# TUI-NICR/EMSANet

Hardware: AMD Instinct MI355X
Metric: images/sec (640x480 RGB-D, bs=32/GPU) fwd+bwd (higher is better)
Workload: dtype f32; 1 GPU; BASELINE.json configs[1]: full EMSANet RGB-D (resnet34-NBt1D x2, SE-add fusion, PPM, semantic+instance+orientation+scene heads), 640x480, bs=32/GPU, f32, train mode (BN batch stats, Dropout2d), step = fwd + bwd (fixed output cotangents) + grad all-reduce + SGD-nesterov update at lr 0 (fixed weights) replayed from a hipGraph; global_batch=32, parallelism=dp1, weights=random init (deterministic), mode=train-hipgraph

## Files before the change

emsanet_amd/_lib.py:

```python
import ctypes
import os
from ctypes import POINTER, Structure, c_char_p, c_float, c_int, c_int8, c_int32, c_int64, c_uint32, c_void_p

LIB_PATH = os.environ.get('EMSA_LIB') or os.path.join(
    os.path.dirname(os.path.abspath(__file__)), 'lib', 'libemsanet_hip.so')


class EmsaPackJob(Structure):
    _fields_ = [('src', c_void_p), ('dst0', c_void_p), ('dst1', c_void_p), ('cout', c_int32),
                ('cin', c_int32), ('kh', c_int32), ('kw', c_int32), ('kind', c_int32),
                ('first_block', c_int32), ('cout_total', c_int32), ('cout_off', c_int32),
                ('cin_total', c_int32), ('cin_off', c_int32)]


class EmsaDropoutJob(Structure):
    _fields_ = [('offset', c_int64), ('c', c_int32), ('layer_id', c_uint32), ('p', c_float),
                ('pad_', c_int32)]


class EmsaConvGeom(Structure):
    _fields_ = [
        ('n_img', c_int32),
        ('in_h', c_int32), ('in_w', c_int32),
        ('out_h', c_int32), ('out_w', c_int32),
# ... 63 lines not shown
    'emsa_bn_bwd_reduce_aff_t': (c_int, [c_int32, _P, _P, _P, _P, _P, _P, c_int32, c_int64, c_int32, _P, _P]),
    'emsa_bn_bwd_apply_aff_t': (c_int, [c_int32, _P, _P, _P, _P, _P, _P, _P, _P, c_int32, c_int32, c_int64,
                                        c_int32, _P, _P, _P, _P]),
    'emsa_conv_wgrad_multi_ws_bytes': (c_int64, [c_int32, c_int32, _GP]),
    'emsa_conv_wgrad_multi_t': (c_int, [c_int32, c_int32, _GP, POINTER(c_void_p), POINTER(c_void_p),
                                        POINTER(c_void_p), POINTER(c_void_p), _P, _P]),
    'emsa_pack_wino': (c_int, [_P, _P, _P, c_int32, c_int32, c_int32, _P]),
    'emsa_pack_batch': (c_int, [_P, c_int32, c_int32, _P]),
    'emsa_conv_wino2d_supported': (c_int, [_GP]),
    'emsa_conv_wino2d_stats_rows': (c_int, [_GP]),
    'emsa_conv_wino2d': (c_int, [_GP, _P, _P, _P, _P, _P, _P, _P, _P, c_int32, _P, c_int32, c_int32, _P]),
    'emsa_pack_wino2d': (c_int, [_P, _P, _P, c_int32, c_int32, _P]),
    'emsa_pack_wino2d_packed': (c_int, [_P, _P, c_int32, c_int32, c_int32, _P]),
    'emsa_pack_wino_packed': (c_int, [_P, _P, c_int32, c_int32, c_int32, c_int32, _P]),
    'emsa_conv_wgrad_ws_bytes': (c_int64, [_GP]),
    'emsa_conv_wgrad': (c_int, [_GP, _P, _P, _P, _P, _P, _P]),
    'emsa_pack_weight_fwd': (c_int, [_P, _P] + [c_int32] * 8 + [_P]),
    'emsa_pack_weight_dgrad': (c_int, [_P, _P] + [c_int32] * 8 + [_P]),
    'emsa_unpack_wgrad': (c_int, [_P, _P] + [c_int32] * 8 + [_P]),
    'emsa_pack_weight_pair': (c_int, [_P, _P, _P] + [c_int32] * 4 + [_P]),
    'emsa_stem_pack_input': (c_int, [_P, _P, c_int32, c_int32, c_int32, c_int32, _P]),
    'emsa_stem_pack_weight': (c_int, [_P, _P, c_int32, c_int32, _P]),
    'emsa_stem_pack_input_rows_t': (c_int, [c_int32, _P, _P, c_int32, c_int32, c_int32, _P]),
    'emsa_stem_pack_weight_rows_t': (c_int, [c_int32, _P, _P, c_int32, _P]),
    'emsa_stem_unpack_wgrad_rows': (c_int, [_P, _P, c_int32, _P]),
    'emsa_stem_unpack_wgrad': (c_int, [_P, _P, c_int32, c_int32, _P]),
    'emsa_bn_finalize': (c_int, [_P, c_int32, c_int32, c_int64, _P, _P, c_float, c_float,
                                 _P, _P, _P, _P, _P, _P, _P, _P]),
    'emsa_bn_finalize_ws_bytes': (c_int, [c_int32]),
    'emsa_bn_fold': (c_int, [_P, _P, _P, _P, c_float, c_int32, _P, _P, _P, _P]),
    'emsa_relu_mask_words': (c_int64, [c_int64]),
    'emsa_bn_act_fwd': (c_int, [_P, _P, _P, _P, _P, _P, c_int32, c_int64, c_int32, c_int32, _P,
                                _P]),
    'emsa_bn_bwd_reduce': (c_int, [_P, _P, _P, _P, _P, _P, _P, c_int32, c_int64, c_int32, c_int32,
                                   _P, _P]),
    'emsa_bn_bwd_rows': (c_int, [c_int64, c_int32]),
    'emsa_bn_bwd_apply': (c_int, [_P, _P, _P, _P, _P, _P, _P, _P, _P, c_int32, c_int32, c_int64,
                                  c_int32, c_int32, c_int32, _P, _P, _P, _P, _P]),
    'emsa_dropout2d_mask': (c_int, [_P, c_int32, c_int32, c_float, c_uint32, c_uint32, _P]),
    'emsa_maxpool3x3s2_fwd': (c_int, [_P, _P, _P, c_int32, c_int32, c_int32, c_int32, _P]),
    'emsa_maxpool3x3s2_bwd': (c_int, [_P, _P, _P, c_int32, c_int32, c_int32, c_int32, _P]),
    'emsa_channel_ws_floats': (c_int, [c_int32, c_int64, c_int32]),
    'emsa_channel_mean': (c_int, [_P, _P, _P, c_int32, c_int64, c_int32, _P]),
    'emsa_se_mlp_fwd': (c_int, [_P] * 7 + [c_int32] * 3 + [_P]),
    'emsa_se_mlp_bwd': (c_int, [_P] * 11 + [c_int32] * 3 + [_P]),
    'emsa_se_scale_add_fwd': (c_int, [_P] * 5 + [c_int32, c_int64, c_int32, _P]),
    'emsa_se_scale_bwd_reduce': (c_int, [_P, _P, _P, _P, c_int32, c_int64, c_int32, _P]),
    'emsa_se_scale_bwd_apply': (c_int, [_P] * 5 + [c_int32, c_int64, c_int32, _P]),
    'emsa_up2x_dw3x3_fwd': (c_int, [_P] * 5 + [c_int32] * 4 + [_P]),
    'emsa_up2x_dw3x3_bwd_data': (c_int, [_P] * 3 + [c_int32] * 4 + [_P]),
    'emsa_up2x_dw3x3_bwd_weight': (c_int, [_P] * 4 + [c_int32] * 4 + [_P]),
    'emsa_up2x_dw3x3_bwd': (c_int, [_P] * 6 + [c_int32] * 4 + [_P]),
    'emsa_up2x_dw3x3_bwd_supported': (c_int, [c_int32, c_int32]),
    'emsa_adaptive_avgpool_fwd': (c_int, [_P, _P] + [c_int32] * 5 + [_P]),
    'emsa_adaptive_avgpool_bwd': (c_int, [_P, _P] + [c_int32] * 6 + [_P]),
    'emsa_bilinear_fwd': (c_int, [_P, _P] + [c_int32] * 7 + [_P]),
    'emsa_bilinear_bwd': (c_int, [_P, _P] + [c_int32] * 7 + [_P]),
    'emsa_head_act_fwd': (c_int, [_P, _P, c_int64] + [c_int32] * 5 + [_P]),
    'emsa_head_act_bwd': (c_int, [_P, _P, _P, _P, c_int64] + [c_int32] * 5 + [_P]),
    'emsa_copy_channels': (c_int, [_P, c_int32, _P, c_int32, c_int64, c_int32, _P]),
    'emsa_axpy': (c_int, [_P, _P, c_int64, c_float, _P]),
    'emsa_ce_semantic_blocks': (c_int, [c_int64]),
    'emsa_ce_semantic_fwd': (c_int, [_P, c_int32, _P, _P, c_int32, c_int64, c_float, c_float, _P, _P,
                                     _P]),
    'emsa_ce_semantic_bwd': (c_int, [_P, c_int32, _P, _P, c_int32, c_int64, c_float, c_float, _P, _P,
                                     _P, c_int32, _P]),
    'emsa_softmax_argmax': (c_int, [_P, c_int32, c_int32, c_int64, _P, _P, _P]),
    'emsa_center_candidates_max': (c_int, []),
    'emsa_center_ws_entries': (c_int64, [c_int32, c_int32, c_int32]),
    'emsa_instance_centers': (c_int, [_P, c_int32, c_int32, c_int32, c_int32, c_int32, c_float,
                                      c_int32, _P, _P, _P, _P, _P, _P, _P, _P]),
    'emsa_instance_assign': (c_int, [_P, c_int32, c_int32, c_int32, c_int32, c_float, c_float, _P,
                                     _P, c_int32, _P, c_float, _P, _P]),
    'emsa_panoptic_merge': (c_int, [_P, _P, _P, c_int32, c_int64, c_int32, c_int32, c_int32, _P, _P,
                                    _P, _P, _P, _P]),
    'emsa_instance_stats': (c_int, [_P, _P, _P, c_int32, c_int64, c_int32, _P, _P, _P]),
    'emsa_panoptic_scores': (c_int, [_P, _P, _P, _P, c_int32, c_int64, c_int32, _P, _P, _P, _P, _P, _P,
                                     _P, _P]),
    'emsa_instance_orientation': (c_int, [_P, c_int32, _P, _P, c_int32, c_int64, c_int32, _P, _P, _P]),
    'emsa_confusion_matrix': (c_int, [_P, c_int32, _P, c_int32, c_int64, c_int32, _P, _P, _P]),
    'emsa_panoptic_targets': (c_int, [_P, c_int32, _P, c_int32, _P, c_int32, c_int64, c_int64, _P, _P]),
    'emsa_panoptic_workspace_bytes': (c_int64, [c_int32, c_int32]),
    'emsa_panoptic_pairs': (c_int, [_P, _P, c_int32, c_int64, c_int32, _P, _P, _P]),
    'emsa_panoptic_match': (c_int, [_P, c_int32, c_int32, c_int32, c_int32, c_int64, _P, _P, _P, _P,
                                    _P, _P]),
    'emsa_panoptic_match_pairs': (c_int, [_P, c_int32, c_int32, c_int32, c_int32, c_int64, _P, _P, _P,
                                          _P, _P, _P, _P, _P]),
    'emsa_angular_error': (c_int, [_P, _P, _P, c_int32, c_int32, _P, c_int32, _P, _P, c_int32, c_int64,
                                   _P, _P, _P]),
    'emsa_export_pack': (c_int, [POINTER(EmsaExportJob), c_int32, c_int32, c_int32, c_int32, _P, _P]),
    'emsa_export_instance_ranks': (c_int, [_P, _P, _P, c_int32, c_int32, c_int32, _P, _P, _P, _P, _P,
                                           _P, _P]),
    'emsa_export_instance_masks': (c_int, [_P, c_int32, c_int32, c_int32, c_int32, c_int32, c_int32,
                                           _P, c_int32, _P, _P, c_int32, _P, _P]),
    'emsa_targets_workspace_bytes': (c_int64, [c_int32, c_int32, c_int32]),
    'emsa_targets_table_entries': (c_int, [c_int32]),
    'emsa_targets_stats': (c_int, [_P, c_int32, _P, c_int32, _P, c_int32, c_int32, c_int32, c_int32, _TP,
                                   c_int32, c_int32, _P, _P]),
    'emsa_targets_finalize': (c_int, [c_int32, c_int32, c_int32, _TP, c_int32, c_int32, _P, _P]),
    'emsa_targets_render': (c_int, [_P, c_int32, _P, c_int32, _P, _P, _P, c_int32, c_int32, c_int32,
                                    c_int32, _TP, c_int32, c_int32, c_int32, _P, _P, _P, _P]),
    'emsa_augment_params': (c_int, [_P, _P] + [c_int32] * 7 + [c_int64, c_float, c_float, c_float, _P]),
    'emsa_augment_apply': (c_int, [_P, _P, _P, c_int32, _P, c_int32, _P] + [c_int32] * 5 +
                           [_P, _P, _P, _P, c_float, _P, _P, c_float, c_float, c_int32, c_int32, _P]),
    'emsa_augment_orientations': (c_int, [_P, _P, _P, c_int32, c_int32, _P]),
    'emsa_normal_l1_blocks': (c_int, [c_int64]),
    'emsa_normal_l1_fwd': (c_int, [_P, c_int32, _P, c_int32, c_int64, c_int64, _P, _P, _P]),
    'emsa_normal_l1_bwd': (c_int, [_P, c_int32, _P, c_int32, c_int64, c_int64, _P, _P, _P, c_int32, _P]),
    'emsa_normal_targets': (c_int, [_P, c_int32, c_int32, c_int32, c_int32, POINTER(EmsaNormalScale),
                                    c_int32, _P]),
    'emsa_augment_normal': (c_int, [_P, c_int32, _P] + [c_int32] * 5 + [_P, _P]),
    'emsa_normal_unit': (c_int, [_P, c_int32, c_int64, _P, _P]),
    'emsa_normal_angular_error': (c_int, [_P, c_int32, c_int32, c_int32, c_int32, _P, c_int32, c_int32,
                                          c_int32, _P, _P, _P]),
    'emsa_normalize_rgb': (c_int, [_P, _P, c_int32, c_int32, c_int32, c_float, _P, _P, _P]),
    'emsa_normalize_depth': (c_int, [_P, _P, c_int64, c_float, c_float, c_int32, _P]),
    'emsa_sgd_nesterov': (c_int, [_P, _P, _P, c_int64, c_float, c_float, c_float, c_float, c_int32,
                                  _P]),
    'emsa_add_t': (c_int, [c_int32, _P, _P, _P, c_int64, _P]),
    'emsa_adam_advance': (c_int, [_P, _P, _P]),
    'emsa_adam_step': (c_int, [_P, _P, _P, _P, c_int64, _P, _P, _P]),
    'emsa_instance_loss_blocks': (c_int, [c_int64]),
    'emsa_instance_loss_fwd': (c_int, [_P, c_int32, _P, c_int32, _P, c_int32, _P, _P, _P, _P, _P, _P,
                                       c_int64, c_float, _P, _P, _P]),
    'emsa_instance_loss_bwd': (c_int, [_P, c_int32, _P, c_int32, _P, c_int32, _P, _P, _P, _P, _P, _P,
                                       c_int64, c_float, _P, _P, _P, c_int32, _P, c_int32, _P,
                                       c_int32, _P]),
    'emsa_bn_act_fwd_t': (c_int, [c_int32, _P, _P, _P, _P, _P, _P, c_int32, c_int64, c_int32, c_int32, _P, _P]),
    'emsa_bn_bwd_reduce_t': (c_int, [c_int32, _P, _P, _P, _P, _P, _P, _P, c_int32, c_int64, c_int32, c_int32, _P, _P]),
    'emsa_bn_bwd_apply_t': (c_int, [c_int32, _P, _P, _P, _P, _P, _P, _P, _P, _P, c_int32, c_int32, c_int64, c_int32, c_int32, c_int32, _P, _P, _P, _P, _P]),
    'emsa_maxpool3x3s2_fwd_t': (c_int, [c_int32, _P, _P, _P, c_int32, c_int32, c_int32, c_int32, _P]),
    'emsa_maxpool3x3s2_bwd_t': (c_int, [c_int32, _P, _P, _P, c_int32, c_int32, c_int32, c_int32, _P]),
    'emsa_se_scale_add_fwd_t': (c_int, [c_int32, _P, _P, _P, _P, _P, c_int32, c_int64, c_int32, _P]),
    'emsa_se_scale_bwd_apply_t': (c_int, [c_int32, _P, _P, _P, _P, _P, c_int32, c_int64, c_int32, _P]),
    'emsa_up2x_dw3x3_fwd_t': (c_int, [c_int32, c_int32, _P, _P, _P, _P, _P, c_int32, c_int32, c_int32, c_int32, _P]),
    'emsa_up2x_dw3x3_bwd_data_t': (c_int, [c_int32, c_int32, _P, _P, _P, c_int32, c_int32, c_int32, c_int32, _P]),
    'emsa_up2x_dw3x3_bwd_weight_t': (c_int, [c_int32, c_int32, _P, _P, _P, _P, c_int32, c_int32, c_int32, c_int32, _P]),
    'emsa_up2x_dw3x3_bwd_t': (c_int, [c_int32, c_int32, _P, _P, _P, _P, _P, _P, c_int32, c_int32, c_int32, c_int32, _P]),
    'emsa_adaptive_avgpool_fwd_t': (c_int, [c_int32, _P, _P, c_int32, c_int32, c_int32, c_int32, c_int32, _P]),
    'emsa_adaptive_avgpool_bwd_t': (c_int, [c_int32, _P, _P, c_int32, c_int32, c_int32, c_int32, c_int32, c_int32, _P]),
    'emsa_bilinear_fwd_t': (c_int, [c_int32, _P, _P, c_int32, c_int32, c_int32, c_int32, c_int32, c_int32, c_int32, _P]),
    'emsa_bilinear_bwd_t': (c_int, [c_int32, _P, _P, c_int32, c_int32, c_int32, c_int32, c_int32, c_int32, c_int32, _P]),
    'emsa_nearest_fwd_t': (c_int, [c_int32, _P, _P, c_int32, c_int32, c_int32, c_int32, c_int32, c_int32, c_int32, _P]),
    'emsa_nearest_bwd_t': (c_int, [c_int32, _P, _P, c_int32, c_int32, c_int32, c_int32, c_int32, c_int32, c_int32, _P]),
    'emsa_head_act_fwd_t': (c_int, [c_int32, c_int32, _P, _P, c_int64, c_int32, c_int32, c_int32, c_int32, c_int32, _P]),
    'emsa_head_act_bwd_gather_t': (c_int, [c_int32, _P, c_int32, c_int32, _P, c_int32, c_int32, _P, c_int32,
                                           c_int32, _P, _P, _P, c_int64, c_int32, c_int32, c_int32, c_int32,
                                           c_int32, _P]),
    'emsa_head_act_bwd_t': (c_int, [c_int32, c_int32, _P, _P, _P, _P, c_int64, c_int32, c_int32, c_int32, c_int32, c_int32, _P]),
    'emsa_stem_pack_input_t': (c_int, [c_int32, _P, _P, c_int32, c_int32, c_int32, c_int32, _P]),
    'emsa_channel_mean_t': (c_int, [c_int32, _P, _P, _P, c_int32, c_int64, c_int32, _P]),
    'emsa_se_pair_fwd_t': (c_int, [c_int32] + [_P] * 14 + [c_int32, c_int64, c_int32, c_int32, _P]),
    'emsa_se_scale_bwd_reduce_t': (c_int, [c_int32, _P, _P, _P, _P, c_int32, c_int64, c_int32, _P]),
    'emsa_cast_channels': (c_int, [c_int32, _P, c_int32, c_int32, _P, c_int32, c_int64, c_int32, _P]),
    'emsa_conv_stats_rows_t': (c_int, [c_int32, _GP]),
    'emsa_conv_igemm_t': (c_int, [c_int32, _GP, _P, _P, _P, _P, _P, _P, _P, _P, c_int32, _P, c_int32,
                                  c_int32, _P]),
    'emsa_conv_wgrad_ws_bytes_t': (c_int64, [c_int32, _GP]),
    'emsa_conv_wgrad_t': (c_int, [c_int32, _GP, _P, _P, _P, _P, _P, _P]),
    'emsa_pack_weight_t': (c_int, [c_int32, _P, _P, _P] + [c_int32] * 8 + [_P]),
    'emsa_conv_igemm_splitk_ws_bytes_t': (c_int64, [c_int32, _GP]),
    'emsa_conv_igemm_splitk_t': (c_int, [c_int32, _GP, _P, _P, _P, _P, _P, _P, _P, c_int32, c_int32, _P, _P]),
    'emsa_up2x_dw3x3_fwd_pair_t': (c_int, [c_int32] + [_P] * 10 + [c_int32] * 4 + [_P]),
    'emsa_conv_igemm_pair_t': (c_int, [c_int32, _GP] + [_P] * 14 + [c_int32, c_int32, _P, _P, _P]),
    'emsa_conv_rs_set_cu_budget': (c_int, [c_int32]),
    'emsa_nbt_half_block_supported': (c_int, [c_int32, c_int32, c_int32]),
    'emsa_nbt_half_block_t': (c_int, [c_int32, c_int32, c_int32, c_int32, c_int32, c_int32,
                                      POINTER(c_void_p), c_int32, POINTER(c_void_p), POINTER(c_void_p),
                                      POINTER(c_void_p), POINTER(c_void_p), POINTER(c_void_p),
                                      POINTER(c_void_p), POINTER(c_void_p), c_int32, POINTER(c_void_p),
                                      c_int32, c_int32, _P]),
    'emsa_conv1d_rs_supported': (c_int, [c_int32, _GP]),
    'emsa_conv1d_rs_stats_rows': (c_int, [c_int32, _GP]),
    'emsa_conv1d_rs_t': (c_int, [c_int32, _GP, _P, _P, _P, _P, _P, _P, _P, _P, c_int32, _P, c_int32,
                                 c_int32, _P]),
    'emsa_conv1d_rs_pair_t': (c_int, [c_int32, _GP] + [_P] * 14 + [c_int32, c_int32, _P]),
    'emsa_conv1d_rs_bnb_t': (c_int, [c_int32, _GP, _P, _P, _P, _P, c_int32, _P, c_int32, _P, _P, _P,
                                     _P, _P, c_int32, _P]),
    'emsa_pack_weight_frag_t': (c_int, [c_int32, _P, _P, _P, c_int32, c_int32, _P]),
    'emsa_stem_pack_weight_t': (c_int, [c_int32, _P, _P, c_int32, c_int32, _P]),
    'emsa_dropout2d_mask_dev': (c_int, [_P, c_int32, c_int32, c_float, _P, c_uint32, _P]),
    'emsa_u32_add': (c_int, [_P, c_uint32, _P]),
    'emsa_sgd_nesterov_dev': (c_int, [_P, _P, _P, c_int64, _P, _P]),
    'emsa_prof_enable': (c_int, [c_int32]),
    'emsa_prof_next_flops': (c_int, [ctypes.c_double]),
    'emsa_prof_reset': (c_int, []),
    'emsa_prof_seen': (c_int, [c_int32]),
    'emsa_prof_name': (c_char_p, [c_int32]),
    'emsa_prof_read': (c_int, [c_int32, POINTER(ctypes.c_double), POINTER(ctypes.c_double),
                               POINTER(c_int32)]),
    'emsa_prof_read_bytes': (c_int, [c_int32, POINTER(ctypes.c_double)]),
}

E_SHAPE = -1
_ERR = {-1: 'EMSA_E_SHAPE (unsupported geometry)', -2: 'EMSA_E_ARG (bad argument)',
        -3: 'EMSA_E_LAUNCH (HIP launch failed)'}


class EmsaError(RuntimeError):
    pass


def _load():
    if not os.path.exists(LIB_PATH):
        raise EmsaError(
            f"{LIB_PATH} not found: build the HIP extension first "
            "(python -c 'import __graft_entry__ as g; g.build()' or make -C emsanet_amd/csrc). "
            "There is no CPU / torch fallback for the EMSANet engine.")
    import torch
    lib = ctypes.CDLL(LIB_PATH)
    for name, (res, args) in SIGNATURES.items():
        fn = getattr(lib, name)
        fn.restype = res
        fn.argtypes = args
    return lib


_lib = None


def lib():
    global _lib
    if _lib is None:
        _lib = _load()
    return _lib


def check(status, name):
    if status != 0:
        raise EmsaError(f"{name} failed: {_ERR.get(status, status)}")
```

emsanet_amd/csrc/pointwise.hip:

```cpp
#include <type_traits>

#include <cstdlib>

#include <atomic>
#include "common.h"

namespace {

constexpr int kThreads = 256;
#ifndef EMSA_PW_BLOCKS_PER_CU
#define EMSA_PW_BLOCKS_PER_CU 8
#endif
constexpr int kMaxBlocks = 256 * EMSA_PW_BLOCKS_PER_CU;

inline int grid_for(long work_items) {
  long b = (work_items + kThreads - 1) / kThreads;
  if (b < 1) b = 1;
  if (b > kMaxBlocks) b = kMaxBlocks;
  return (int)b;
}

__global__ void pack_weight_kernel(const float* __restrict__ src, float* __restrict__ dst, int cout,
                                   int cin, int kh, int kw, int cout_total, int cout_off,
                                   int cin_total, int cin_off, int mode,
                                   float* __restrict__ dst2 = nullptr) {
  const long total = (long)cout * cin * kh * kw;
  const int taps = kh * kw;
  for (long i = blockIdx.x * (long)blockDim.x + threadIdx.x; i < total;
       i += (long)gridDim.x * blockDim.x) {
    const int tap = (int)(i % taps);
    const long r = i / taps;
    const int ci = (int)(r % cin), co = (int)(r / cin);
    if (mode == 3) {
      const float v = src[i];
      dst[((long)tap * cout_total + cout_off + co) * cin_total + cin_off + ci] = v;
      dst2[((long)tap * cin_total + cin_off + ci) * cout_total + cout_off + co] = v;
    } else if (mode == 0) {
      dst[((long)tap * cout_total + cout_off + co) * cin_total + cin_off + ci] = src[i];
    } else if (mode == 1) {
      dst[((long)tap * cin_total + cin_off + ci) * cout_total + cout_off + co] = src[i];
    } else {
      dst[i] = src[((long)tap * cout_total + cout_off + co) * cin_total + cin_off + ci];
    }
  }
}

template <typename T>
__global__ void pack_weight_t_kernel(const float* __restrict__ src, T* __restrict__ dst,
                                     T* __restrict__ dst2, int cout, int cin, int taps,
                                     int cout_total, int cout_off, int cin_total, int cin_off) {
  const long total = (long)cout * cin * taps;
  for (long i = blockIdx.x * (long)blockDim.x + threadIdx.x; i < total;
       i += (long)gridDim.x * blockDim.x) {
    const int tap = (int)(i % taps);
    const long r = i / taps;
    const int ci = (int)(r % cin), co = (int)(r / cin);
    const float v = src[i];
    if (dst) emsa_st1(dst + ((long)tap * cout_total + cout_off + co) * cin_total + cin_off + ci, v);
    if (dst2) emsa_st1(dst2 + ((long)tap * cin_total + cin_off + ci) * cout_total + cout_off + co, v);
  }
}

template <typename T>
__global__ void stem_pack_input_kernel(const float* __restrict__ x, T* __restrict__ y, int n,
                                       int c, int h, int w) {
  const int wp = w + 8;
  const long total = (long)n * h * wp;
  for (long i = blockIdx.x * (long)blockDim.x + threadIdx.x; i < total;
       i += (long)gridDim.x * blockDim.x) {
    const int col = (int)(i % wp);
    const long r = i / wp;
    const int row = (int)(r % h), img = (int)(r / h);
    const int sw = col - 3;
    float4 v = emsa_zero4();
    if (sw >= 0 && sw < w) {
      const long base = ((long)img * c * h + row) * w + sw;
      const long plane = (long)h * w;
      v.x = x[base];
      if (c > 1) v.y = x[base + plane];
      if (c > 2) v.z = x[base + 2 * plane];
      if (c > 3) v.w = x[base + 3 * plane];
    }
    emsa_st4(y + i * 4, v);
  }
}

template <typename T>
__global__ void stem_pack_input_rows_kernel(const float* __restrict__ x, T* __restrict__ y, int n,
                                            int h, int w) {
  const int wp = w + 8, hp = h + 4;
  const long total = (long)n * hp * wp;
  for (long i = blockIdx.x * (long)blockDim.x + threadIdx.x; i < total;
       i += (long)gridDim.x * blockDim.x) {
    const int col = (int)(i % wp);
    const long r = i / wp;
    const int row = (int)(r % hp), img = (int)(r / hp);
    const int sw = col - 3;
    float v[4] = {0.f, 0.f, 0.f, 0.f};
    if (sw >= 0 && sw < w) {
#pragma unroll
      for (int k = 0; k < 4; ++k) {
        const int sr = row - 3 + k;
        if (sr >= 0 && sr < h) v[k] = x[((long)img * h + sr) * w + sw];
      }
    }
    emsa_st4(y + i * 4, make_float4(v[0], v[1], v[2], v[3]));
  }
}
template <typename T>
__global__ void stem_pack_weight_rows_kernel(const float* __restrict__ w, T* __restrict__ wp,
                                             int cout, int unpack) {
  const int total = 2 * cout * 32;
  for (int i = blockIdx.x * blockDim.x + threadIdx.x; i < total; i += gridDim.x * blockDim.x) {
    const int k = i % 32, co = (i / 32) % cout, t = i / (32 * cout);
    const int kw = k / 4, kh = 4 * t + (k % 4);
    const bool real = kw < 7 && kh < 7;
    if (!unpack) {
      emsa_st1(wp + i, real ? w[(co * 7 + kh) * 7 + kw] : 0.f);
    } else if (real) {
      emsa_st1(wp + (co * 7 + kh) * 7 + kw, w[i]);
    }
  }
}

template <typename T>
__global__ void stem_pack_weight_kernel(const float* __restrict__ w, T* __restrict__ wp,
                                        int cout, int cin, int unpack) {
  const int total = 7 * cout * 32;
  for (int i = blockIdx.x * blockDim.x + threadIdx.x; i < total; i += gridDim.x * blockDim.x) {
    const int k = i % 32, co = (i / 32) % cout, kh = i / (32 * cout);
    const int kw = k / 4, c = k % 4;
    const bool real = kw < 7 && c < cin;
    if (!unpack) {
      emsa_st1(wp + i, real ? w[((co * cin + c) * 7 + kh) * 7 + kw] : 0.f);
    } else if (real) {
      emsa_st1(wp + ((co * cin + c) * 7 + kh) * 7 + kw, w[i]);
    }
  }
}

constexpr int kBnSlices = 64;
__global__ void bn_partial_kernel(const float* __restrict__ stats, int rows, int c,
                                  double* __restrict__ ws) {
  __shared__ double sh[3][8][32];
  const int cl = threadIdx.x & 31, rg = threadIdx.x >> 5;
  const int ch = blockIdx.x * 32 + cl;
  const int slices = gridDim.y, sl = blockIdx.y;
  const int per = (rows + slices - 1) / slices;
  const int r0 = sl * per, r1 = min(r0 + per, rows);
  double s0 = 0.0, s1 = 0.0, q = 0.0;
  if (ch < c)
    for (int r = r0 + rg; r < r1; r += 8) {
      const double nb = (double)stats[((long)2 * rows + r) * c + ch];
      if (nb > 0.0) {
        const double sb = (double)stats[((long)0 * rows + r) * c + ch];
        s0 += nb;
        s1 += sb;
        q += (double)stats[((long)1 * rows + r) * c + ch] + sb * sb / nb;
      }
    }
  sh[0][rg][cl] = s0; sh[1][rg][cl] = s1; sh[2][rg][cl] = q;
  __syncthreads();
  if (rg == 0 && ch < c) {
    s0 = s1 = q = 0.0;
#pragma unroll
    for (int k = 0; k < 8; ++k) { s0 += sh[0][k][cl]; s1 += sh[1][k][cl]; q += sh[2][k][cl]; }
    double* o = ws + ((long)sl * c + ch) * 3;
    o[0] = s0; o[1] = s1; o[2] = q;
  }
}

__global__ void bn_finalize_kernel(const double* __restrict__ ws, int slices, int c,
                                   const float* __restrict__ gamma, const float* __restrict__ beta,
                                   float eps, float momentum, float* running_mean,
                                   float* running_var, float* __restrict__ scale,
                                   float* __restrict__ shift, float* __restrict__ save_mean,
                                   float* __restrict__ save_invstd) {
  __shared__ double sh[3][8][32];
  const int cl = threadIdx.x & 31, rg = threadIdx.x >> 5;
  const int ch = blockIdx.x * 32 + cl;
  double n = 0.0, s1 = 0.0, q = 0.0;
  if (ch < c)
    for (int sl = rg; sl < slices; sl += 8) {
      const double* o = ws + ((long)sl * c + ch) * 3;
      n += o[0]; s1 += o[1]; q += o[2];
    }
  sh[0][rg][cl] = n; sh[1][rg][cl] = s1; sh[2][rg][cl] = q;
  __syncthreads();
  if (rg != 0 || ch >= c) return;
  n = s1 = q = 0.0;
#pragma unroll
  for (int k = 0; k < 8; ++k) { n += sh[0][k][cl]; s1 += sh[1][k][cl]; q += sh[2][k][cl]; }
  const double mean = n > 0.0 ? s1 / n : 0.0;
  double m2 = q - s1 * mean;
  if (m2 < 0.0) m2 = 0.0;
  const double var = n > 0.0 ? m2 / n : 0.0;
  const float invstd = (float)(1.0 / sqrt(var + (double)eps));
  const float sc = gamma[ch] * invstd;
  scale[ch] = sc;
  shift[ch] = beta[ch] - (float)mean * sc;
  save_mean[ch] = (float)mean;
  save_invstd[ch] = invstd;
  if (running_mean) {
    const double unbiased = n > 1.0 ? m2 / (n - 1.0) : var;
    running_mean[ch] = (1.f - momentum) * running_mean[ch] + momentum * (float)mean;
    running_var[ch] = (1.f - momentum) * running_var[ch] + momentum * (float)unbiased;
  }
}

template <int RG>
__global__ __launch_bounds__(4 * RG) void bn_finalize_rows_kernel(const float* __restrict__ stats, int rows, int c,
                                        const float* __restrict__ gamma, const float* __restrict__ beta,
                                        float eps, float momentum, float* running_mean,
                                        float* running_var, float* __restrict__ scale,
                                        float* __restrict__ shift, float* __restrict__ save_mean,
                                        float* __restrict__ save_invstd) {
  __shared__ double sh[3][RG][4];
  const int cl = threadIdx.x & 3, rg = threadIdx.x >> 2;
  const int ch = blockIdx.x * 4 + cl;
  const int chc = ch < c ? ch : c - 1;
  double n = 0.0, s1 = 0.0, q = 0.0;
#pragma unroll 8
  for (int r = rg; r < rows; r += RG) {
    const float nbf = stats[((long)2 * rows + r) * c + chc];
    const float sbf = stats[((long)0 * rows + r) * c + chc];
    const float m2f = stats[((long)1 * rows + r) * c + chc];
    const double nb = (double)nbf, sb = (double)sbf;
    const bool ok = nbf > 0.f;
    n += ok ? nb : 0.0;
    s1 += ok ? sb : 0.0;
    const double r0 = (double)(1.0f / (ok ? nbf : 1.f));
    const double rn = r0 * (2.0 - (ok ? nb : 1.0) * r0);
    q += ok ? (double)m2f + sb * sb * rn : 0.0;
  }
#pragma unroll
  for (int off = 4; off < 64; off <<= 1) {
    n += __shfl_xor(n, off);
    s1 += __shfl_xor(s1, off);
    q += __shfl_xor(q, off);
  }
  constexpr int NW = 4 * RG / 64;
  const int wv = threadIdx.x >> 6;
  if ((threadIdx.x & 63) < 4) { sh[0][wv][cl] = n; sh[1][wv][cl] = s1; sh[2][wv][cl] = q; }
  __syncthreads();
  if (rg != 0 || ch >= c) return;
  n = s1 = q = 0.0;
#pragma unroll
  for (int k = 0; k < NW; ++k) { n += sh[0][k][cl]; s1 += sh[1][k][cl]; q += sh[2][k][cl]; }
  const double mean = n > 0.0 ? s1 / n : 0.0;
  double m2 = q - s1 * mean;
  if (m2 < 0.0) m2 = 0.0;
  const double var = n > 0.0 ? m2 / n : 0.0;
  const float invstd = (float)(1.0 / sqrt(var + (double)eps));
  const float sc = gamma[ch] * invstd;
  scale[ch] = sc;
  shift[ch] = beta[ch] - (float)mean * sc;
  save_mean[ch] = (float)mean;
  save_invstd[ch] = invstd;
  if (running_mean) {
    const double unbiased = n > 1.0 ? m2 / (n - 1.0) : var;
    running_mean[ch] = (1.f - momentum) * running_mean[ch] + momentum * (float)mean;
    running_var[ch] = (1.f - momentum) * running_var[ch] + momentum * (float)unbiased;
  }
}

__global__ void bn_fold_kernel(const float* gamma, const float* beta, const float* rm,
                               const float* rv, float eps, int c, float* scale, float* shift,
                               float* invstd) {
  const int i = blockIdx.x * blockDim.x + threadIdx.x;
  if (i < c) {
    const float is = 1.0f / sqrtf(rv[i] + eps);
    const float sc = gamma[i] * is;
    scale[i] = sc;
    shift[i] = beta[i] - rm[i] * sc;
    if (invstd) invstd[i] = is;
  }
}

__device__ __forceinline__ float bn_mul(float a, float b) {
#pragma clang fp contract(off)
  return a * b;
}
__device__ __forceinline__ float bn_add(float a, float b) {
#pragma clang fp contract(off)
  return a + b;
}
__device__ __forceinline__ float bn_affine(float x, float sc, float sh) { return __builtin_fmaf(x, sc, sh); }
__device__ __forceinline__ float bn_acc_xhat(float acc, float g, float x, float mu, float is) {
  return __builtin_fmaf(bn_mul(g, bn_add(x, -mu)), is, acc);
}
__device__ __forceinline__ float bn_dx_train(float g, float x, float mu, float is, float gi, float db,
                                             float dg, float inv_count) {
  const float xh = bn_mul(bn_add(x, -mu), is);
  const float t = __builtin_fmaf(-db, inv_count, g);
  return bn_mul(gi, __builtin_fmaf(-bn_mul(xh, dg), inv_count, t));
}

template <typename T> struct VecIO {
  static constexpr int V = 8;
  typedef typename std::conditional<std::is_same<T, emsa_f16>::value, _Float16, __bf16>::type E;
  typedef E ev __attribute__((ext_vector_type(8)));
  typedef float fv __attribute__((ext_vector_type(8)));
  static __device__ __forceinline__ void load(const T* p, float (&v)[8]) {
    const fv f = __builtin_convertvector(*reinterpret_cast<const ev*>(p), fv);
#pragma unroll
    for (int k = 0; k < 8; ++k) v[k] = f[k];
  }
  typedef ev raw;
  static __device__ __forceinline__ raw load_raw(const T* p) { return *reinterpret_cast<const ev*>(p); }
  static __device__ __forceinline__ void cvt(const raw& r, float (&v)[8]) {
    const fv f = __builtin_convertvector(r, fv);
#pragma unroll
    for (int k = 0; k < 8; ++k) v[k] = f[k];
  }
  static __device__ __forceinline__ void store(T* p, const float (&v)[8]) {
    fv f;
#pragma unroll
    for (int k = 0; k < 8; ++k) f[k] = v[k];
    *reinterpret_cast<ev*>(p) = __builtin_convertvector(f, ev);
  }
};
template <> struct VecIO<float> {
  static constexpr int V = 4;
  static __device__ __forceinline__ void load(const float* p, float (&v)[4]) {
    const float4 f = emsa_ld4(p);
    v[0] = f.x; v[1] = f.y; v[2] = f.z; v[3] = f.w;
  }
  typedef float4 raw;
  static __device__ __forceinline__ raw load_raw(const float* p) { return emsa_ld4(p); }
  static __device__ __forceinline__ void cvt(const raw& f, float (&v)[4]) {
    v[0] = f.x; v[1] = f.y; v[2] = f.z; v[3] = f.w;
  }
  static __device__ __forceinline__ void store(float* p, const float (&v)[4]) {
    emsa_st4(p, make_float4(v[0], v[1], v[2], v[3]));
  }
};
template <int V>
__device__ __forceinline__ void ldf(const float* p, float (&v)[V]) {
#pragma unroll
  for (int k = 0; k < V; k += 4) {
    const float4 f = emsa_ld4(p + k);
    v[k] = f.x; v[k + 1] = f.y; v[k + 2] = f.z; v[k + 3] = f.w;
  }
}

template <typename T>
__global__ void bn_act_fwd_kernel(const T* __restrict__ x, T* __restrict__ y,
                                  const float* __restrict__ scale, const float* __restrict__ shift,
                                  const float* __restrict__ drop,
                                  const T* __restrict__ residual, long hw, int cvn, long totalv,
                                  int act, uint64_t* __restrict__ mask_bits) {
  constexpr int V = VecIO<T>::V;
  for (long i = blockIdx.x * (long)blockDim.x + threadIdx.x; i < totalv;
       i += (long)gridDim.x * blockDim.x) {
    const int cv = (int)(i % cvn);
    const long pix = i / cvn;
    float v[V], sc[V], sh[V];
    VecIO<T>::load(x + i * V, v);
    ldf<V>(scale + cv * V, sc);
    ldf<V>(shift + cv * V, sh);
#pragma unroll
    for (int k = 0; k < V; ++k) v[k] = bn_affine(v[k], sc[k], sh[k]);
    if (drop) {
      float d[V];
      ldf<V>(drop + (pix / hw) * (long)cvn * V + cv * V, d);
#pragma unroll
      for (int k = 0; k < V; ++k) v[k] = bn_mul(v[k], d[k]);
    }
    if (residual) {
      float r[V];
      VecIO<T>::load(residual + i * V, r);
#pragma unroll
      for (int k = 0; k < V; ++k) v[k] = bn_add(v[k], r[k]);
    }
    if (act == EMSA_ACT_RELU) {
#pragma unroll
      for (int k = 0; k < V; ++k) v[k] = fmaxf(v[k], 0.f);
    }
    VecIO<T>::store(y + i * V, v);
    if (mask_bits) {
      uint64_t b[V];
#pragma unroll
      for (int k = 0; k < V; ++k) b[k] = __ballot(v[k] > 0.f);
      if ((i & 63) == 0) {
        uint64_t* m = mask_bits + (i >> 6) * V;
#pragma unroll
        for (int k = 0; k < V; ++k) m[k] = b[k];
      }
    }
  }
}

template <typename T, bool DROP, bool RES>
__global__ __launch_bounds__(kThreads) void bn_act_fwd_fast_kernel(
    const T* __restrict__ x, T* __restrict__ y, const float* __restrict__ scale,
    const float* __restrict__ shift, const float* __restrict__ drop, const T* __restrict__ residual,
    uint32_t hw, int cvn_log2, uint32_t totalv, int act, uint64_t* __restrict__ mask_bits) {
  constexpr int V = VecIO<T>::V;
  typedef typename VecIO<T>::raw Raw;
  const uint32_t stride = gridDim.x * kThreads;
  uint32_t i = blockIdx.x * kThreads + threadIdx.x;
  const uint32_t cvn = 1u << cvn_log2, cv = i & (cvn - 1);
  const uint32_t dpix = stride >> cvn_log2;
  uint32_t pix = i >> cvn_log2;
  float sc[V], sh[V];
  ldf<V>(scale + cv * V, sc);
  ldf<V>(shift + cv * V, sh);
  auto finish = [&](uint32_t idx, const Raw& rx, const Raw& rr, const float (&d)[V]) {
    float v[V];
    VecIO<T>::cvt(rx, v);
#pragma unroll
    for (int k = 0; k < V; ++k) v[k] = bn_affine(v[k], sc[k], sh[k]);
    if constexpr (DROP) {
#pragma unroll
      for (int k = 0; k < V; ++k) v[k] = bn_mul(v[k], d[k]);
    }
    if constexpr (RES) {
      float r[V];
      VecIO<T>::cvt(rr, r);
#pragma unroll
      for (int k = 0; k < V; ++k) v[k] = bn_add(v[k], r[k]);
    }
    if (act == EMSA_ACT_RELU) {
#pragma unroll
      for (int k = 0; k < V; ++k) v[k] = fmaxf(v[k], 0.f);
    }
    VecIO<T>::store(y + (size_t)idx * V, v);
    if (mask_bits) {
      uint64_t b[V];
#pragma unroll
      for (int k = 0; k < V; ++k) b[k] = __ballot(v[k] > 0.f);
      if ((idx & 63) == 0) {
        uint64_t* m = mask_bits + (size_t)(idx >> 6) * V;
#pragma unroll
        for (int k = 0; k < V; ++k) m[k] = b[k];
      }
    }
  };
  auto ld_drop = [&](uint32_t px, float (&d)[V]) {
    if constexpr (DROP) ldf<V>(drop + ((size_t)(px / hw) * cvn + cv) * V, d);
  };
  uint32_t iw = i & ~63u;
  for (; iw + stride + 64 <= totalv; iw += 2 * stride, i += 2 * stride, pix += 2 * dpix) {
    const uint32_t i1 = i + stride;
    const Raw x0 = VecIO<T>::load_raw(x + (size_t)i * V);
    const Raw x1 = VecIO<T>::load_raw(x + (size_t)i1 * V);
    Raw r0 = x0, r1 = x1;
    if constexpr (RES) {
// ... 2325 lines not shown
    case EMSA_DT_F32: { return maxpool3x3s2_fwd_impl<float>((const float*)x, (float*)y, idx, n, h, w, c, stream); }
    case EMSA_DT_BF16: { return maxpool3x3s2_fwd_impl<emsa_bf16>((const emsa_bf16*)x, (emsa_bf16*)y, idx, n, h, w, c, stream); }
    case EMSA_DT_F16: { return maxpool3x3s2_fwd_impl<emsa_f16>((const emsa_f16*)x, (emsa_f16*)y, idx, n, h, w, c, stream); }
    default: return EMSA_E_ARG;
  }
}
template <typename T>
static int maxpool3x3s2_bwd_impl(const T* dy, const int8_t* idx, T* dx, int32_t n, int32_t h, int32_t w, int32_t c, void* stream) {
  if (!dy || !dx || !idx) return EMSA_E_ARG;
  if (!cv_ok<T>(c)) return EMSA_E_SHAPE;
  constexpr int V = VecIO<T>::V;
  const long total = (long)n * ((h + 1) / 2) * ((w + 1) / 2) * (c / V);
  if (idx32_ok((long)n * h * w * c))
    hipLaunchKernelGGL((maxpool_bwd_kernel<T, uint32_t>), dim3(grid_for(total)), dim3(kThreads), 0,
                       (hipStream_t)stream, dy, idx, dx, n, h, w, c / V);
  else
    hipLaunchKernelGGL((maxpool_bwd_kernel<T, long>), dim3(grid_for(total)), dim3(kThreads), 0,
                       (hipStream_t)stream, dy, idx, dx, n, h, w, c / V);
  return emsa_launch_status();
}
extern "C" int emsa_maxpool3x3s2_bwd(const float* dy, const int8_t* idx, float* dx, int32_t n, int32_t h, int32_t w, int32_t c, void* stream) {
  return maxpool3x3s2_bwd_impl<float>(dy, idx, dx, n, h, w, c, stream);
}
extern "C" int emsa_maxpool3x3s2_bwd_t(int32_t dtype, const void* dy, const int8_t* idx, void* dx, int32_t n, int32_t h, int32_t w, int32_t c, void* stream) {
  switch (dtype) {
    case EMSA_DT_F32: { return maxpool3x3s2_bwd_impl<float>((const float*)dy, idx, (float*)dx, n, h, w, c, stream); }
    case EMSA_DT_BF16: { return maxpool3x3s2_bwd_impl<emsa_bf16>((const emsa_bf16*)dy, idx, (emsa_bf16*)dx, n, h, w, c, stream); }
    case EMSA_DT_F16: { return maxpool3x3s2_bwd_impl<emsa_f16>((const emsa_f16*)dy, idx, (emsa_f16*)dx, n, h, w, c, stream); }
    default: return EMSA_E_ARG;
  }
}

static std::atomic<int> g_batch_invariant{0};
static int channel_splits(long hw, int n) {
  int splits = (int)((hw + 511) / 512);
  if (splits > 64) splits = 64;
  if ((long)n * splits <= 64 && !g_batch_invariant.load(std::memory_order_relaxed)) {
    splits = (int)((hw + 63) / 64);
    if (splits > 256) splits = 256;
  }
  if (splits < 1) splits = 1;
  return splits;
}

extern "C" int emsa_set_batch_invariant(int on) {
  return g_batch_invariant.exchange(on ? 1 : 0, std::memory_order_relaxed);
}

template <typename T>
static int channel_dot(const T* a, const T* b, float* out, float* ws, int n, long hw,
                       int c, float scale, hipStream_t st) {
  if (!cv_ok<T>(c)) return EMSA_E_SHAPE;
  const int splits = channel_splits(hw, n);
  const int cvn = c / VecIO<T>::V;
  if (cvn > kThreads) {
    const dim3 grid(n * splits, (cvn + kThreads - 1) / kThreads);
    if (b)
      hipLaunchKernelGGL((channel_dot_wide_kernel<T, true>), grid, dim3(kThreads), 0, st, a, b, ws, hw,
                         cvn, splits);
    else
      hipLaunchKernelGGL((channel_dot_wide_kernel<T, false>), grid, dim3(kThreads), 0, st, a, b, ws, hw,
                         cvn, splits);
    hipLaunchKernelGGL(channel_dot_finish_kernel, dim3((n * c + 255) / 256), dim3(256), 0, st, ws,
                       out, n, c, splits, scale);
    return emsa_launch_status();
  }
  const int lanes = kThreads / cvn;
  const size_t lds = (size_t)lanes * c * sizeof(float);
  if (b)
    hipLaunchKernelGGL((channel_dot_kernel<T, true>), dim3(n * splits), dim3(kThreads), lds, st, a, b,
                       ws, hw, cvn, splits);
  else
    hipLaunchKernelGGL((channel_dot_kernel<T, false>), dim3(n * splits), dim3(kThreads), lds, st, a, b,
                       ws, hw, cvn, splits);
  hipLaunchKernelGGL(channel_dot_finish_kernel, dim3((n * c + 255) / 256), dim3(256), 0, st, ws,
                     out, n, c, splits, scale);
  return emsa_launch_status();
}

extern "C" int emsa_channel_ws_floats(int32_t n, int64_t hw, int32_t c) {
  return n * channel_splits((long)hw, n) * c;
}
extern "C" int emsa_channel_mean(const float* x, float* gap, float* ws, int32_t n, int64_t hw,
                                 int32_t c, void* stream) {
  if (!x || !gap || !ws) return EMSA_E_ARG;
  return channel_dot<float>(x, nullptr, gap, ws, n, (long)hw, c, 1.0f / (float)hw,
                            (hipStream_t)stream);
}
extern "C" int emsa_channel_mean_t(int32_t dtype, const void* x, float* gap, float* ws, int32_t n,
                                   int64_t hw, int32_t c, void* stream) {
  if (!x || !gap || !ws) return EMSA_E_ARG;
  EMSA_DISPATCH_DTYPE(dtype, T, return channel_dot<T>((const T*)x, (const T*)nullptr, gap, ws, n,
                                                      (long)hw, c, 1.0f / (float)hw,
                                                      (hipStream_t)stream));
  return EMSA_E_ARG;
}
extern "C" int emsa_se_scale_bwd_reduce(const float* dout, const float* x, float* ds, float* ws,
                                        int32_t n, int64_t hw, int32_t c, void* stream) {
  if (!dout || !x || !ds || !ws) return EMSA_E_ARG;
  return channel_dot<float>(dout, x, ds, ws, n, (long)hw, c, 1.0f, (hipStream_t)stream);
}
extern "C" int emsa_se_scale_bwd_reduce_t(int32_t dtype, const void* dout, const void* x, float* ds,
                                          float* ws, int32_t n, int64_t hw, int32_t c,
                                          void* stream) {
  if (!dout || !x || !ds || !ws) return EMSA_E_ARG;
  EMSA_DISPATCH_DTYPE(dtype, T, return channel_dot<T>((const T*)dout, (const T*)x, ds, ws, n,
                                                      (long)hw, c, 1.0f, (hipStream_t)stream));
  return EMSA_E_ARG;
}

extern "C" int emsa_se_mlp_fwd(const float* gap, const float* w1, const float* b1,
                               const float* w2, const float* b2, float* hid, float* s, int32_t n,
                               int32_t c, int32_t cr, void* stream) {
  if (!gap || !w1 || !b1 || !w2 || !b2 || !hid || !s) return EMSA_E_ARG;
  hipLaunchKernelGGL(se_mlp_fwd_kernel, dim3(n), dim3(256), (size_t)(c + cr) * sizeof(float),
                     (hipStream_t)stream, gap, w1, b1, w2, b2, hid, s, c, cr);
  return emsa_launch_status();
}
template <typename T>
static int se_pair_fwd(const T* xa, const T* xb, float* ws, const float* const* wts, float* gap,
                       float* hid, float* s, int n, long hw, int c, int cr, hipStream_t st) {
  if (!cv_ok<T>(c)) return EMSA_E_SHAPE;
  const int splits = channel_splits(hw, n);
  const int cvn = c / VecIO<T>::V;
  if (cvn > kThreads) {
    hipLaunchKernelGGL((channel_dot_wide_kernel<T, false>),
                       dim3(2 * n * splits, (cvn + kThreads - 1) / kThreads), dim3(kThreads), 0, st, xa,
                       (const T*)nullptr, ws, hw, cvn, splits, xb, n * splits);
  } else {
    const int lanes = kThreads / cvn;
    const size_t lds = (size_t)lanes * c * sizeof(float);
    hipLaunchKernelGGL((channel_dot_kernel<T, false>), dim3(2 * n * splits), dim3(kThreads), lds, st, xa,
                       (const T*)nullptr, ws, hw, cvn, splits, xb, n * splits);
  }
  hipLaunchKernelGGL(se_mlp_pair_fwd_kernel, dim3(2 * n), dim3(256),
                     (size_t)(c + cr) * sizeof(float), st, ws, splits, 1.0f / (float)hw, wts[0],
                     wts[1], wts[2], wts[3], wts[4], wts[5], wts[6], wts[7], gap, hid, s, n, c, cr);
  return emsa_launch_status();
}
extern "C" int emsa_se_pair_fwd_t(int32_t dtype, const void* xa, const void* xb, float* ws,
                                  const float* w1a, const float* b1a, const float* w2a,
                                  const float* b2a, const float* w1b, const float* b1b,
                                  const float* w2b, const float* b2b, float* gap, float* hid,
                                  float* s, int32_t n, int64_t hw, int32_t c, int32_t cr,
                                  void* stream) {
  if (!xa || !xb || !ws || !w1a || !b1a || !w2a || !b2a || !w1b || !b1b || !w2b || !b2b || !gap ||
      !hid || !s)
    return EMSA_E_ARG;
  const float* wts[8] = {w1a, b1a, w2a, b2a, w1b, b1b, w2b, b2b};
  EMSA_DISPATCH_DTYPE(dtype, T, return se_pair_fwd<T>((const T*)xa, (const T*)xb, ws, wts, gap, hid,
                                                      s, n, (long)hw, c, cr, (hipStream_t)stream));
  return EMSA_E_ARG;
}
extern "C" int emsa_se_mlp_bwd(const float* gap, const float* w1, const float* w2,
                               const float* hid, const float* s, const float* ds, float* dgap,
                               float* dw1, float* db1, float* dw2, float* db2, int32_t n,
                               int32_t c, int32_t cr, void* stream) {
  if (!gap || !w1 || !w2 || !hid || !s || !ds || !dgap || !dw1 || !db1 || !dw2 || !db2)
    return EMSA_E_ARG;
  hipStream_t st = (hipStream_t)stream;
  if (n <= c && cr <= 32 && cr >= 1) {
    float* dz1 = dw2;
    const size_t lds = (size_t)(c + (256 / cr) * cr + cr) * sizeof(float);
    hipLaunchKernelGGL(se_mlp_bwd_a_kernel, dim3(n), dim3(256), lds, st, w1, w2, hid, s, ds, dgap,
                       dz1, c, cr);
    const int wblocks = (c * cr + 255) / 256;
    hipLaunchKernelGGL(se_mlp_bwd_w_kernel<0>, dim3(wblocks + (cr + 255) / 256), dim3(256), 0, st,
                       gap, hid, s, ds, dz1, dw1, db1, n, c, cr, wblocks);
    hipLaunchKernelGGL(se_mlp_bwd_w_kernel<1>, dim3(wblocks + (c + 255) / 256), dim3(256), 0, st,
                       gap, hid, s, ds, dz1, dw2, db2, n, c, cr, wblocks);
    return emsa_launch_status();
  }
  if ((size_t)n * cr * sizeof(float) > 60000) return EMSA_E_SHAPE;
  hipLaunchKernelGGL(se_mlp_bwd_kernel, dim3(8), dim3(256), (size_t)n * cr * sizeof(float), st, gap,
                     w1, w2, hid, s, ds, dgap, dw1, db1, dw2, db2, n, c, cr);
  return emsa_launch_status();
}

template <typename T>
static int se_scale_add_fwd_impl(const T* a, const float* sa, const T* b, const float* sb, T* out, int32_t n, int64_t hw, int32_t c, void* stream) {
  if (!a || !sa || !out || ((b == nullptr) != (sb == nullptr))) return EMSA_E_ARG;
  if (!cv_ok<T>(c)) return EMSA_E_SHAPE;
  const long totalv = (long)n * hw * (c / VecIO<T>::V);
  const dim3 grid(grid_for(totalv)), block(kThreads);
  hipStream_t st = (hipStream_t)stream;
  const int cvn = c / VecIO<T>::V;
#define EMSA_SE_FWD(B, I)                                                                          \
  hipLaunchKernelGGL((se_scale_add_fwd_kernel<T, B, I>), grid, block, 0, st, a, sa, b, sb, out,   \
                     (I)hw, cvn, (I)totalv)
  if (idx32_ok((long)n * hw * c)) {
    if (b) EMSA_SE_FWD(true, uint32_t); else EMSA_SE_FWD(false, uint32_t);
  } else {
    if (b) EMSA_SE_FWD(true, long); else EMSA_SE_FWD(false, long);
  }
#undef EMSA_SE_FWD
  return emsa_launch_status();
}
extern "C" int emsa_se_scale_add_fwd(const float* a, const float* sa, const float* b, const float* sb, float* out, int32_t n, int64_t hw, int32_t c, void* stream) {
  return se_scale_add_fwd_impl<float>(a, sa, b, sb, out, n, hw, c, stream);
}
extern "C" int emsa_se_scale_add_fwd_t(int32_t dtype, const void* a, const float* sa, const void* b, const float* sb, void* out, int32_t n, int64_t hw, int32_t c, void* stream) {
  switch (dtype) {
    case EMSA_DT_F32: { return se_scale_add_fwd_impl<float>((const float*)a, sa, (const float*)b, sb, (float*)out, n, hw, c, stream); }
    case EMSA_DT_BF16: { return se_scale_add_fwd_impl<emsa_bf16>((const emsa_bf16*)a, sa, (const emsa_bf16*)b, sb, (emsa_bf16*)out, n, hw, c, stream); }
    case EMSA_DT_F16: { return se_scale_add_fwd_impl<emsa_f16>((const emsa_f16*)a, sa, (const emsa_f16*)b, sb, (emsa_f16*)out, n, hw, c, stream); }
    default: return EMSA_E_ARG;
  }
}
template <typename T>
static int se_scale_bwd_apply_impl(const T* dout, const float* s, const float* dgap, const T* dx_extra, T* dx, int32_t n, int64_t hw, int32_t c, void* stream) {
  if (!dout || !s || !dgap || !dx) return EMSA_E_ARG;
  if (!cv_ok<T>(c)) return EMSA_E_SHAPE;
  const long totalv = (long)n * hw * (c / VecIO<T>::V);
  const dim3 grid(grid_for(totalv)), block(kThreads);
  hipStream_t st = (hipStream_t)stream;
  const int cvn = c / VecIO<T>::V;
  const float inv_hw = 1.0f / (float)hw;
#define EMSA_SE_BWD(E, I)                                                                          \
  hipLaunchKernelGGL((se_scale_bwd_apply_kernel<T, E, I>), grid, block, 0, st, dout, s, dgap,     \
                     dx_extra, dx, (I)hw, cvn, (I)totalv, inv_hw)
  if (idx32_ok((long)n * hw * c)) {
    if (dx_extra) EMSA_SE_BWD(true, uint32_t); else EMSA_SE_BWD(false, uint32_t);
  } else {
    if (dx_extra) EMSA_SE_BWD(true, long); else EMSA_SE_BWD(false, long);
  }
#undef EMSA_SE_BWD
  return emsa_launch_status();
}
extern "C" int emsa_se_scale_bwd_apply(const float* dout, const float* s, const float* dgap, const float* dx_extra, float* dx, int32_t n, int64_t hw, int32_t c, void* stream) {
  return se_scale_bwd_apply_impl<float>(dout, s, dgap, dx_extra, dx, n, hw, c, stream);
}
extern "C" int emsa_se_scale_bwd_apply_t(int32_t dtype, const void* dout, const float* s, const float* dgap, const void* dx_extra, void* dx, int32_t n, int64_t hw, int32_t c, void* stream) {
  switch (dtype) {
    case EMSA_DT_F32: { return se_scale_bwd_apply_impl<float>((const float*)dout, s, dgap, (const float*)dx_extra, (float*)dx, n, hw, c, stream); }
    case EMSA_DT_BF16: { return se_scale_bwd_apply_impl<emsa_bf16>((const emsa_bf16*)dout, s, dgap, (const emsa_bf16*)dx_extra, (emsa_bf16*)dx, n, hw, c, stream); }
    case EMSA_DT_F16: { return se_scale_bwd_apply_impl<emsa_f16>((const emsa_f16*)dout, s, dgap, (const emsa_f16*)dx_extra, (emsa_f16*)dx, n, hw, c, stream); }
    default: return EMSA_E_ARG;
  }
}

template <typename T, typename TO>
static int up2x_dw3x3_fwd_impl(const T* x, const float* wdw, const float* bias, const T* skip, TO* y, int32_t n, int32_t h, int32_t w, int32_t c, void* stream) {
  if (!x || !wdw || !y) return EMSA_E_ARG;
  if (!c4_ok(c)) return EMSA_E_SHAPE;
  const long total = (long)n * 4 * h * w * (c / 4);
  static const int nt_env = [] {
    const char* e = getenv("EMSA_UP2X_NT");
    return e ? (e[0] == '1' ? 1 : 0) : -1;
  }();
  const bool nt = nt_env >= 0 ? nt_env == 1 : c >= 32;
  const dim3 grid(grid_for(total)), block(kThreads);
  const size_t lds = (size_t)9 * c * sizeof(float);
  hipStream_t st = (hipStream_t)stream;
#define EMSA_UP_FWD(NTF, I)                                                                         \
  do {                                                                                              \
    if (skip)                                                                                       \
      hipLaunchKernelGGL((up2x_dw_fwd_kernel<T, TO, NTF, I, true>), grid, block, lds, st, x, wdw,   \
                         bias, skip, y, n, h, w, c / 4);                                            \
    else                                                                                            \
      hipLaunchKernelGGL((up2x_dw_fwd_kernel<T, TO, NTF, I, false>), grid, block, lds, st, x, wdw,  \
                         bias, skip, y, n, h, w, c / 4);                                            \
  } while (0)
  const bool i32 = idx32_ok((long)n * 4 * h * w * c);
  if (nt && std::is_same<TO, float>::value) {
    if (i32) EMSA_UP_FWD(true, uint32_t); else EMSA_UP_FWD(true, long);
  } else {
    if (i32) EMSA_UP_FWD(false, uint32_t); else EMSA_UP_FWD(false, long);
  }
#undef EMSA_UP_FWD
  return emsa_launch_status();
}
template <typename T>
static int up2x_pair_impl(const T* x0, const T* x1, const float* w0, const float* w1, const float* b0,
                          const float* b1, const T* s0, const T* s1, T* y0, T* y1, int n, int h,
                          int w, int c, hipStream_t st) {
  const long total = (long)n * 4 * h * w * (c / 4);
  if ((s0 == nullptr) != (s1 == nullptr)) return EMSA_E_ARG;
#define EMSA_UP_PAIR(I, SK)                                                                         \
  hipLaunchKernelGGL((up2x_dw_fwd_kernel<T, T, false, I, SK>), dim3(grid_for(total), 2),            \
                     dim3(kThreads), (size_t)9 * c * sizeof(float), st, x0, w0, b0, s0, y0, n, h, w, \
                     c / 4, x1, w1, b1, s1, y1)
  if (idx32_ok((long)n * 4 * h * w * c)) {
    if (s0) EMSA_UP_PAIR(uint32_t, true); else EMSA_UP_PAIR(uint32_t, false);
  } else {
    if (s0) EMSA_UP_PAIR(long, true); else EMSA_UP_PAIR(long, false);
  }
#undef EMSA_UP_PAIR
  return emsa_launch_status();
}
extern "C" int emsa_up2x_dw3x3_fwd_pair_t(int32_t dtype, const void* x0, const void* x1,
                                          const float* wdw0, const float* wdw1, const float* bias0,
                                          const float* bias1, const void* skip0, const void* skip1,
                                          void* y0, void* y1, int32_t n, int32_t h, int32_t w,
                                          int32_t c, void* stream) {
  if (!x0 || !x1 || !wdw0 || !wdw1 || !y0 || !y1 || y0 == y1) return EMSA_E_ARG;
  if ((bias0 == nullptr) != (bias1 == nullptr) || (skip0 == nullptr) != (skip1 == nullptr))
    return EMSA_E_ARG;
  if (!c4_ok(c)) return EMSA_E_SHAPE;
  hipStream_t st = (hipStream_t)stream;
  if (dtype == EMSA_DT_BF16)
    return up2x_pair_impl<emsa_bf16>((const emsa_bf16*)x0, (const emsa_bf16*)x1, wdw0, wdw1, bias0, bias1,
                                     (const emsa_bf16*)skip0, (const emsa_bf16*)skip1, (emsa_bf16*)y0,
                                     (emsa_bf16*)y1, n, h, w, c, st);
  if (dtype == EMSA_DT_F16)
    return up2x_pair_impl<emsa_f16>((const emsa_f16*)x0, (const emsa_f16*)x1, wdw0, wdw1, bias0, bias1,
                                    (const emsa_f16*)skip0, (const emsa_f16*)skip1, (emsa_f16*)y0,
// ... 457 lines not shown
```

emsanet_amd/functional.py:

```python
import ctypes
import os

import torch

from . import _lib
from ._lib import EmsaConvGeom, check

ACT_NONE, ACT_RELU = 0, 1


def _stream():
    return torch.cuda.current_stream().cuda_stream


_POISON = bool(os.environ.get('EMSA_POISON'))


def _empty(shape, device, dtype=torch.float32):
    t = torch.empty(shape, device=device, dtype=dtype)
    if _POISON:
        t.fill_(float('nan') if dtype.is_floating_point else 111)
    return t


# ... 990 lines not shown
    y = act_empty(n, c, h, w, x.device, dtype=x.dtype)
    L = _lib.lib()
    bits = None
    if want_mask and act == ACT_RELU:
        bits = torch.empty(L.emsa_relu_mask_words(n * c * h * w), device=x.device,
                           dtype=torch.int64)
    check(call_t('emsa_bn_act_fwd', dt(x), _p(x), _p(y), _p(scale), _p(shift), _p(drop),
                 _p(residual), n, h * w, c, act, _p(bits), _stream()), 'emsa_bn_act_fwd')
    return (y, bits) if want_mask else y


def bn_bwd(dy, y, x, gamma, mean, invstd, drop, act, train, want_dres, dg_out=None, db_out=None):
    n, c, h, w = x.shape
    assert ld_of(x) == c and ld_of(dy) == c and dy.dtype == x.dtype
    L = _lib.lib()
    code = dt(x)
    bits = None
    if y is not None and y.dtype == torch.int64:
        y, bits = None, y
    rows = L.emsa_bn_bwd_rows(n * h * w, c)
    partial = _empty((2, rows, c), x.device)
    check(call_t('emsa_bn_bwd_reduce', code, _p(dy), _p(y), _p(bits), _p(x), _p(mean), _p(invstd),
                 _p(drop), n, h * w, c, act, _p(partial), _stream()), 'emsa_bn_bwd_reduce')
    dx = act_empty(n, c, h, w, x.device, dtype=x.dtype)
    dres = act_empty(n, c, h, w, x.device, dtype=x.dtype) if want_dres else None
    if dg_out is None or db_out is None:
        dgb = _empty((2, c), x.device)
        dg_out, db_out = dgb[0], dgb[1]
    check(call_t('emsa_bn_bwd_apply', code, _p(dy), _p(y), _p(bits), _p(x), _p(gamma), _p(mean),
                 _p(invstd), _p(drop), _p(partial), rows, n, h * w, c, act, 1 if train else 0,
                 _p(dx), _p(dres), _p(dg_out), _p(db_out), _stream()), 'emsa_bn_bwd_apply')
    return dx, dres, dg_out, db_out


def dropout2d_mask(n, c, p, seed, layer_id, device):
    m = _empty((n, c), device)
    if torch.is_tensor(seed):
        check(_lib.lib().emsa_dropout2d_mask_dev(_p(m), n, c, p, _p(seed), layer_id, _stream()),
              'emsa_dropout2d_mask_dev')
    else:
        check(_lib.lib().emsa_dropout2d_mask(_p(m), n, c, p, seed & 0xFFFFFFFF, layer_id,
                                             _stream()), 'emsa_dropout2d_mask')
    return m


def dropout2d_mask_batch(jobs_dev, n_jobs, total_floats, n, max_c, seed, device):
    m = _empty((total_floats,), device)
    if torch.is_tensor(seed):
        check(_lib.lib().emsa_dropout2d_mask_batch(_p(m), _p(jobs_dev), n_jobs, n, max_c, 0, _p(seed),
                                                   _stream()), 'emsa_dropout2d_mask_batch')
    else:
        check(_lib.lib().emsa_dropout2d_mask_batch(_p(m), _p(jobs_dev), n_jobs, n, max_c,
                                                   seed & 0xFFFFFFFF, None, _stream()),
              'emsa_dropout2d_mask_batch')
    return m


def maxpool_fwd(x):
    n, c, h, w = x.shape
    assert ld_of(x) == c
    oh, ow = (h + 1) // 2, (w + 1) // 2
    y = act_empty(n, c, oh, ow, x.device, dtype=x.dtype)
    idx = _empty((n, oh, ow, c), x.device, torch.int8)
    check(call_t('emsa_maxpool3x3s2_fwd', dt(x), _p(x), _p(y), _p(idx), n, h, w, c, _stream()),
          'emsa_maxpool3x3s2_fwd')
    return y, idx


def maxpool_bwd(dy, idx, in_hw):
    n, c = dy.shape[:2]
    h, w = in_hw
    assert ld_of(dy) == c
    dx = act_empty(n, c, h, w, dy.device, dtype=dy.dtype)
    check(call_t('emsa_maxpool3x3s2_bwd', dt(dy), _p(dy), _p(idx), _p(dx), n, h, w, c, _stream()),
          'emsa_maxpool3x3s2_bwd')
    return dx


def channel_mean(x):
    n, c, h, w = x.shape
    assert ld_of(x) == c
    gap = _empty((n, c), x.device)
    ws = _empty((_lib.lib().emsa_channel_ws_floats(n, h * w, c),), x.device)
    check(call_t('emsa_channel_mean', dt(x), _p(x), _p(gap), _p(ws), n, h * w, c, _stream()),
          'emsa_channel_mean')
    return gap


def se_mlp_fwd(gap, w1, b1, w2, b2):
    n, c = gap.shape
    cr = w1.shape[0]
    hid = _empty((n, cr), gap.device)
    s = _empty((n, c), gap.device)
    check(_lib.lib().emsa_se_mlp_fwd(_p(gap), _p(w1), _p(b1), _p(w2), _p(b2), _p(hid), _p(s), n, c,
                                     cr, _stream()), 'emsa_se_mlp_fwd')
    return hid, s


def se_pair_fwd(xa, xb, wa, wb):
    n, c, h, w = xa.shape
    assert xb.shape == xa.shape and xb.dtype == xa.dtype and ld_of(xa) == c and ld_of(xb) == c
    cr = wa[0].shape[0]
    dev = xa.device
    gap, hid, s = _empty((2, n, c), dev), _empty((2, n, cr), dev), _empty((2, n, c), dev)
    ws = _empty((2 * _lib.lib().emsa_channel_ws_floats(n, h * w, c),), dev)
    check(_lib.lib().emsa_se_pair_fwd_t(dt(xa), _p(xa), _p(xb), _p(ws), _p(wa[0]), _p(wa[1]),
                                        _p(wa[2]), _p(wa[3]), _p(wb[0]), _p(wb[1]), _p(wb[2]),
                                        _p(wb[3]), _p(gap), _p(hid), _p(s), n, h * w, c, cr,
                                        _stream()), 'emsa_se_pair_fwd_t')
    return gap[0], gap[1], hid[0], hid[1], s[0], s[1]


def se_mlp_bwd(gap, w1, w2, hid, s, ds):
    n, c = gap.shape
    cr = w1.shape[0]
    dev = gap.device
    dgap = _empty((n, c), dev)
    dw1 = _empty((cr, c), dev)
    db1 = _empty((cr,), dev)
    dw2 = _empty((c, cr), dev)
    db2 = _empty((c,), dev)
    check(_lib.lib().emsa_se_mlp_bwd(_p(gap), _p(w1), _p(w2), _p(hid), _p(s), _p(ds), _p(dgap),
                                     _p(dw1), _p(db1), _p(dw2), _p(db2), n, c, cr, _stream()),
          'emsa_se_mlp_bwd')
    return dgap, dw1, db1, dw2, db2


def se_scale_add(a, sa, b=None, sb=None):
    n, c, h, w = a.shape
    out = act_empty(n, c, h, w, a.device, dtype=a.dtype)
    check(call_t('emsa_se_scale_add_fwd', dt(a), _p(a), _p(sa), _p(b), _p(sb), _p(out), n, h * w,
                 c, _stream()), 'emsa_se_scale_add_fwd')
    return out


def se_scale_bwd_reduce(dout, x):
    n, c, h, w = x.shape
    assert dout.dtype == x.dtype
    ds = _empty((n, c), x.device)
    ws = _empty((_lib.lib().emsa_channel_ws_floats(n, h * w, c),), x.device)
    check(call_t('emsa_se_scale_bwd_reduce', dt(x), _p(dout), _p(x), _p(ds), _p(ws), n, h * w, c,
                 _stream()), 'emsa_se_scale_bwd_reduce')
    return ds


def se_scale_bwd_apply(dout, s, dgap, extra=None):
    n, c, h, w = dout.shape
    dx = act_empty(n, c, h, w, dout.device, dtype=dout.dtype)
    check(call_t('emsa_se_scale_bwd_apply', dt(dout), _p(dout), _p(s), _p(dgap), _p(extra), _p(dx),
                 n, h * w, c, _stream()), 'emsa_se_scale_bwd_apply')
    return dx


def _two(name, feat, out_f32, *args):
    code = dt(feat)
    L = _lib.lib()
    if code == 0:
        return getattr(L, name)(*args)
    return getattr(L, name + '_t')(code, 1 if out_f32 else 0, *args)


def up2x_dw_fwd(x, wdw, bias, skip=None, out_f32=False):
    n, c, h, w = x.shape
    assert ld_of(x) == c and (skip is None or (ld_of(skip) == c and skip.dtype == x.dtype))
    y = act_empty(n, c, 2 * h, 2 * w, x.device,
                  dtype=torch.float32 if out_f32 else x.dtype)
    check(_two('emsa_up2x_dw3x3_fwd', x, out_f32, _p(x), _p(wdw), _p(bias), _p(skip), _p(y), n, h,
               w, c, _stream()), 'emsa_up2x_dw3x3_fwd')
    return y


UP2X_FUSED_BWD = os.environ.get('EMSA_UP2X_FUSED', '1') != '0'


def up2x_dw_fwd_pair(xs, wdws, biases, skips):
    x0, x1 = xs
    if x0.dtype == torch.float32 or x0.dtype != x1.dtype or x0.shape != x1.shape:
        return None
    if (biases[0] is None) != (biases[1] is None) or (skips[0] is None) != (skips[1] is None):
        return None
    n, c, h, w = x0.shape
    for t in (x0, x1) + tuple(k for k in skips if k is not None):
        if ld_of(t) != c or t.dtype != x0.dtype:
            return None
    y0 = act_empty(n, c, 2 * h, 2 * w, x0.device, dtype=x0.dtype)
    y1 = act_empty(n, c, 2 * h, 2 * w, x0.device, dtype=x0.dtype)
    check(_lib.lib().emsa_up2x_dw3x3_fwd_pair_t(
        dt(x0), _p(x0), _p(x1), _p(wdws[0]), _p(wdws[1]), _p(biases[0]), _p(biases[1]), _p(skips[0]),
        _p(skips[1]), _p(y0), _p(y1), n, h, w, c, _stream()), 'emsa_up2x_dw3x3_fwd_pair_t')
    return y0, y1


def up2x_dw_bwd(dy, x, wdw, need_dx=True):
    n, c, h, w = x.shape
    assert ld_of(dy) == c
    out_f32 = dy.dtype == torch.float32
    if not out_f32 and dy.dtype != x.dtype:
        raise _lib.EmsaError(f"up-sampling gradient {dy.dtype} for {x.dtype} features")
    dx = act_empty(n, c, h, w, x.device, dtype=x.dtype) if need_dx else None
    dwb = torch.zeros(c * 10, device=x.device, dtype=torch.float32)
    dw, db = dwb[:c * 9], dwb[c * 9:]
    if UP2X_FUSED_BWD and _lib.lib().emsa_up2x_dw3x3_bwd_supported(c, x.element_size()):
        check(_two('emsa_up2x_dw3x3_bwd', x, out_f32, _p(dy), _p(x), _p(wdw), _p(dx), _p(dw), _p(db),
                   n, h, w, c, _stream()), 'emsa_up2x_dw3x3_bwd')
        return dx, dw, db
    if need_dx:
        check(_two('emsa_up2x_dw3x3_bwd_data', x, out_f32, _p(dy), _p(wdw), _p(dx), n, h, w, c,
                   _stream()), 'emsa_up2x_dw3x3_bwd_data')
    check(_two('emsa_up2x_dw3x3_bwd_weight', x, out_f32, _p(dy), _p(x), _p(dw), _p(db), n, h, w, c,
               _stream()), 'emsa_up2x_dw3x3_bwd_weight')
    return dx, dw, db


def adaptive_avgpool_fwd(x, bins):
    n, c, h, w = x.shape
    assert ld_of(x) == c
    y = act_empty(n, c, bins, bins, x.device, dtype=x.dtype)
    check(call_t('emsa_adaptive_avgpool_fwd', dt(x), _p(x), _p(y), n, h, w, c, bins, _stream()),
          'emsa_adaptive_avgpool_fwd')
    return y


def adaptive_avgpool_bwd(dy, dx, bins, accumulate):
    n, c, h, w = dx.shape
    assert dy.dtype == dx.dtype
    check(call_t('emsa_adaptive_avgpool_bwd', dt(dx), _p(dy), _p(dx), n, h, w, c, bins,
                 1 if accumulate else 0, _stream()), 'emsa_adaptive_avgpool_bwd')
    return dx


def bilinear_fwd(x, out):
    n, c, ih, iw = x.shape
    oh, ow = out.shape[2:]
    assert ld_of(x) == c and out.dtype == x.dtype
    check(call_t('emsa_bilinear_fwd', dt(x), _p(x), _p(out), n, ih, iw, oh, ow, c, ld_of(out),
                 _stream()), 'emsa_bilinear_fwd')
    return out


def bilinear_bwd(dy, in_hw):
    n, c, oh, ow = dy.shape
    ih, iw = in_hw
    dx = act_empty(n, c, ih, iw, dy.device)
    check(call_t('emsa_bilinear_bwd', dt(dy), _p(dy), _p(dx), n, ih, iw, oh, ow, c, ld_of(dy),
                 _stream()), 'emsa_bilinear_bwd')
    if dy.dtype != torch.float32:
        dx = cast(dx, dy.dtype)
    return dx


def nearest_fwd(x, out):
    n, c, ih, iw = x.shape
    oh, ow = out.shape[2:]
    assert ld_of(x) == c and out.dtype == x.dtype
    check(_lib.lib().emsa_nearest_fwd_t(dt(x), _p(x), _p(out), n, ih, iw, oh, ow, c, ld_of(out),
                                        _stream()), 'emsa_nearest_fwd_t')
    return out


def nearest_bwd(dy, in_hw):
    n, c, oh, ow = dy.shape
    ih, iw = in_hw
    dx = act_empty(n, c, ih, iw, dy.device)
    check(_lib.lib().emsa_nearest_bwd_t(dt(dy), _p(dy), _p(dx), n, ih, iw, oh, ow, c, ld_of(dy),
                                        _stream()), 'emsa_nearest_bwd_t')
    if dy.dtype != torch.float32:
        dx = cast(dx, dy.dtype)
    return dx


def add(a, b):
    assert a.shape == b.shape and a.dtype == b.dtype and ld_of(a) == a.shape[1] == ld_of(b)
    n, c, h, w = a.shape
    out = act_empty(n, c, h, w, a.device, dtype=a.dtype)
    check(_lib.lib().emsa_add_t(dt(a), _p(a), _p(b), _p(out), a.numel(), _stream()), 'emsa_add_t')
    return out


def head_act_fwd(x, n_sig, n_tanh, n_norm=0, norm_off=3):
    n, c, h, w = x.shape
    assert ld_of(x) == c
    y = act_empty(n, c, h, w, x.device)
    check(_two('emsa_head_act_fwd', x, True, _p(x), _p(y), n * h * w, c, n_sig, n_tanh, norm_off,
               n_norm, _stream()), 'emsa_head_act_fwd')
    return y


def head_act_bwd(dy, y, n_sig, n_tanh, n_norm=0, x=None, norm_off=3, dtype=torch.float32):
    n, c, h, w = y.shape
    assert ld_of(dy) == c and dy.dtype == torch.float32 and y.dtype == torch.float32
    dx = act_empty(n, c, h, w, y.device, dtype=dtype)
    check(_two('emsa_head_act_bwd', dx, True, _p(dy), _p(y), _p(x), _p(dx), n * h * w, c, n_sig,
               n_tanh, norm_off, n_norm, _stream()), 'emsa_head_act_bwd')
    return dx


HEAD_GATHER = os.environ.get('EMSA_HEAD_GATHER', '1') != '0'


def head_act_bwd_gather(grads, sizes, y, n_sig, n_tanh, n_norm=0, x=None, norm_off=3,
                        dtype=torch.float32):
    n, c, h, w = y.shape
    if c != 8 or len(sizes) > 3 or y.dtype != torch.float32 or ld_of(y) != c or not HEAD_GATHER:
        return None
    gs = []
    for g_ in grads:
# ... 41 lines not shown
```

emsanet_amd/nn.py:

```python
import os

import torch
import torch.nn as nn

from . import functional as Fn
from . import ops
from .functional import ACT_NONE, ACT_RELU


class Spec:
    BLOCK_BN_EPS = 1e-3
    DEFAULT_BN_EPS = 1e-5
    BN_MOMENTUM = 0.1
    SE_REDUCTION = 16
    PPM_BINS = (1, 5)
    STEM_BIAS = False
    DW_UPSAMPLE_BIAS = True
    SIDE_OUTPUT_KERNEL = 1
    SKIP_FUSION_1X1 = True
    ORIENTATION_L2_NORMALIZE = False
    RESNET_LAYERS = {'resnet18': (2, 2, 2, 2), 'resnet34': (3, 4, 6, 3), 'resnet50': (3, 4, 6, 3),
                     'resnet101': (3, 4, 23, 3)}


# ... 2 lines not shown


class ConvNormAct(nn.Module):

    def __init__(self, cin, cout, kernel_size, stride=1, act=True, eps=Spec.DEFAULT_BN_EPS):
        super().__init__()
        self.conv = nn.Conv2d(cin, cout, kernel_size, stride=stride, padding=kernel_size // 2,
                              bias=False)
        self.norm = nn.BatchNorm2d(cout, eps=eps, momentum=Spec.BN_MOMENTUM)
        self.act = ACT_RELU if act else ACT_NONE
        self._crt, self._brt = ops.ConvRT(self.conv), ops.BNRT(self.norm)

    def forward(self, x):
        if _fast_eval(self):
            return ops.conv_bn_act_eval(Fn.as_act(x), self._crt, self._brt, self.act)
        return ops.ConvBNActFunction.apply(x, self._crt, self._brt, self.act, self.conv.weight,
                                           self.norm.weight, self.norm.bias)


class Dropout2dHash(nn.Module):

    def __init__(self, p):
        super().__init__()
        self.p = float(p)
        self.layer_id = -1
        self.seed_fn = lambda: 0

    def mask(self, n, c, device):
        if not self.training or self.p == 0.0:
            return None
        pre = getattr(self, '_premade', None)
        if pre is not None and pre.shape == (n, c) and pre.device == device:
            self._premade = None
            return pre
        return Fn.dropout2d_mask(n, c, self.p, self.seed_fn(), self.layer_id, device)


class NonBottleneck1D(nn.Module):
    def __init__(self, cin, cout, stride=1, dropout_p=0.0):
        super().__init__()
        self.conv3x1_1 = nn.Conv2d(cin, cout, (3, 1), stride=(stride, 1), padding=(1, 0))
        self.conv1x3_1 = nn.Conv2d(cout, cout, (1, 3), stride=(1, stride), padding=(0, 1))
        self.bn1 = nn.BatchNorm2d(cout, eps=Spec.BLOCK_BN_EPS, momentum=Spec.BN_MOMENTUM)
        self.conv3x1_2 = nn.Conv2d(cout, cout, (3, 1), padding=(1, 0))
        self.conv1x3_2 = nn.Conv2d(cout, cout, (1, 3), padding=(0, 1))
        self.bn2 = nn.BatchNorm2d(cout, eps=Spec.BLOCK_BN_EPS, momentum=Spec.BN_MOMENTUM)
        self.dropout = Dropout2dHash(dropout_p)
        if stride != 1 or cin != cout:
            self.downsample = nn.Sequential(
                nn.Conv2d(cin, cout, 1, stride=stride, bias=False),
                nn.BatchNorm2d(cout, eps=Spec.DEFAULT_BN_EPS, momentum=Spec.BN_MOMENTUM))
        else:
            self.downsample = None
        self._rt = ops.NBt1DRT(self)

    def forward(self, x):
        if _fast_eval(self):
            return ops.nbt1d_eval(Fn.as_act(x, dense=True), self._rt)
        drop = self.dropout.mask(x.shape[0], self.conv1x3_2.out_channels, x.device)
        return ops.NBt1DFunction.apply(x, self._rt, drop, *self._rt.params())


class _ResidualBlock(nn.Module):

    def _add(self, name, cin, cout, k, stride=1):
        conv = nn.Conv2d(cin, cout, k, stride=stride, padding=k // 2, bias=False)
        bn = nn.BatchNorm2d(cout, eps=Spec.DEFAULT_BN_EPS, momentum=Spec.BN_MOMENTUM)
        setattr(self, f'conv{name}', conv)
        setattr(self, f'bn{name}', bn)
        rt = (ops.ConvRT(conv), ops.BNRT(bn), conv, bn)
        self._crts.append(rt[0])
        return rt

    def _finish(self, cin, cout, stride):
        if stride != 1 or cin != cout:
            self.downsample = nn.Sequential(
                nn.Conv2d(cin, cout, 1, stride=stride, bias=False),
                nn.BatchNorm2d(cout, eps=Spec.DEFAULT_BN_EPS, momentum=Spec.BN_MOMENTUM))
            self._ds = (ops.ConvRT(self.downsample[0]), ops.BNRT(self.downsample[1]),
                        self.downsample[0], self.downsample[1])
            self._crts.append(self._ds[0])
        else:
            self.downsample, self._ds = None, None

    def forward(self, x):
        fast = _fast_eval(self)
        x = Fn.as_act(x, dense=True) if fast else x
        y = x
        for crt, brt, conv, bn in self._chain[:-1]:
            y = ops.conv_bn_act_eval(y, crt, brt, ACT_RELU) if fast else \
                ops.ConvBNActFunction.apply(y, crt, brt, ACT_RELU, conv.weight, bn.weight, bn.bias)
        idn = x
        if self._ds is not None:
            crt, brt, conv, bn = self._ds
            idn = ops.conv_bn_act_eval(x, crt, brt, ACT_NONE) if fast else \
                ops.ConvBNActFunction.apply(x, crt, brt, ACT_NONE, conv.weight, bn.weight, bn.bias)
        crt, brt, conv, bn = self._chain[-1]
        if fast:
            return ops.conv_bn_act_eval(y, crt, brt, ACT_RELU, residual=idn)
        return ops.ConvBNAddActFunction.apply(y, idn, crt, brt, ACT_RELU, conv.weight, bn.weight,
                                              bn.bias)


class BasicBlock(_ResidualBlock):
    expansion = 1

    def __init__(self, cin, c, stride=1, dropout_p=0.0):
        super().__init__()
        self._crts = []
        self._chain = [self._add('1', cin, c, 3, stride), self._add('2', c, c, 3)]
        self._finish(cin, c, stride)


class Bottleneck(_ResidualBlock):
    expansion = 4

    def __init__(self, cin, c, stride=1, dropout_p=0.0):
        super().__init__()
        self._crts = []
        self._chain = [self._add('1', cin, c, 1), self._add('2', c, c, 3, stride),
                       self._add('3', c, 4 * c, 1)]
        self._finish(cin, 4 * c, stride)


RESNET_BLOCKS = {'nonbottleneck1d': None, 'basicblock': BasicBlock, 'bottleneck': Bottleneck}


class ResNetNBt1D(nn.Module):

    def __init__(self, name, n_input_channels, dropout_p, block='nonbottleneck1d'):
        super().__init__()
        if name not in Spec.RESNET_LAYERS:
            raise NotImplementedError(f"backbone '{name}' (ResNet-18/34/101 layouts)")
        if block not in RESNET_BLOCKS:
            raise NotImplementedError(f"resnet block '{block}'")
        layers = Spec.RESNET_LAYERS[name]
        self.conv1 = nn.Conv2d(n_input_channels, 64, 7, stride=2, padding=3, bias=Spec.STEM_BIAS)
        self.bn1 = nn.BatchNorm2d(64, eps=Spec.DEFAULT_BN_EPS, momentum=Spec.BN_MOMENTUM)
        cin = 64
        cls = RESNET_BLOCKS[block] or NonBottleneck1D
        exp = getattr(cls, 'expansion', 1)
        for i, (c, n) in enumerate(zip((64, 128, 256, 512), layers)):
            blocks = []
            for j in range(n):
                blocks.append(cls(cin, c, stride=2 if (i > 0 and j == 0) else 1,
                                  dropout_p=dropout_p))
                cin = c * exp
            setattr(self, f'layer{i + 1}', nn.Sequential(*blocks))
        self.stage_channels = (64, 64 * exp, 128 * exp, 256 * exp, 512 * exp)
        self.stage_downsamplings = (2, 4, 8, 16, 32)
        self._stem = ops.StemRT(self.conv1, self.bn1)
        self.compute_dtype = torch.float32

    def forward_stage(self, i, x):
        if i == 0:
            if _fast_eval(self):
                return ops.stem_eval(x, self._stem, self.compute_dtype)
            return ops.StemFunction.apply(x, self._stem, self.conv1.weight, self.bn1.weight,
                                          self.bn1.bias, self.conv1.bias, self.compute_dtype)
        if i == 1:
            x = ops.MaxPoolFunction.apply(x)
        return getattr(self, f'layer{i}')(x)


class SqueezeAndExcitation(nn.Module):
    def __init__(self, c):
        super().__init__()
        self.fc = nn.Sequential(nn.Conv2d(c, c // Spec.SE_REDUCTION, 1), nn.ReLU(),
                                nn.Conv2d(c // Spec.SE_REDUCTION, c, 1), nn.Sigmoid())


class SEAddUniRGB(nn.Module):

    def __init__(self, c):
        super().__init__()
        self.se_rgb = SqueezeAndExcitation(c)
        self.se_depth = SqueezeAndExcitation(c)

    def forward(self, rgb, depth):
        ps = ops._se_params(self.se_rgb) + ops._se_params(self.se_depth)
        return ops.SEAddFunction.apply(rgb, depth, *ps)


_DUAL_ENV = os.environ.get('EMSA_DUAL_STREAM')
DUAL_STREAM = None


def _dual_stream(t):
    if t is None or not t.is_cuda or not torch.cuda.is_available():
        return False
    if DUAL_STREAM is not None:
        return DUAL_STREAM
    if _DUAL_ENV is not None:
        return _DUAL_ENV != '0'
    return True


_TWIN_ENV = os.environ.get('EMSA_TWIN')
TWIN = None


TWIN_MAX_PIXELS = 3 * 640 * 480


def twin_launches(t=None):
    if TWIN is not None:
        return TWIN
    if _TWIN_ENV is not None:
        return _TWIN_ENV != '0'
    return t is None or t.shape[0] * t.shape[2] * t.shape[3] <= TWIN_MAX_PIXELS


class CutPlan:

    DECODERS = 99
    DECODER_MID = 98

    def __init__(self, stages=(2, 1), decoder_cut=False):
        self.stages = tuple(sorted(set(int(s) for s in stages), reverse=True))
        if any(s < 0 or s > 3 for s in self.stages):
            raise ValueError("CutPlan: encoder cuts go after stage 0..3")
        self.decoder_cut = bool(decoder_cut)
        self.records = []
        self.late_stages = set()

    def begin(self):
        self.records = []

    def cut(self, t, stage, group):
        c = t.detach().requires_grad_(True)
        self.records.append((t, c, stage, group))
        return c


class FusedEncoder(nn.Module):

    def __init__(self, backbone_rgb, backbone_depth, fusion, skip_downsamplings,
                 backbone_rgbd=None):
        super().__init__()
        self.backbone_rgb = backbone_rgb
        self.backbone_depth = backbone_depth
        self.backbone_rgbd = backbone_rgbd
        if backbone_rgbd is not None and (backbone_rgb is not None or backbone_depth is not None):
            raise ValueError("input modality 'rgbd' excludes 'rgb' and 'depth'")
        bb = backbone_rgb if backbone_rgb is not None else backbone_depth
        bb = bb if bb is not None else backbone_rgbd
        self.two = backbone_rgb is not None and backbone_depth is not None
        if self.two:
            if fusion != 'se-add-uni-rgb':
                raise NotImplementedError(f"encoder fusion '{fusion}'")
            self.fusion_modules = nn.ModuleList([SEAddUniRGB(c) for c in bb.stage_channels])
        self.skip_downsamplings = tuple(skip_downsamplings)
        self._side_stream = None
        self.downsampling = 32
        self.n_channels_out = bb.stage_channels[-1]
        ch = dict(zip(bb.stage_downsamplings, bb.stage_channels))
        self.skips_n_channels = tuple(ch[d] for d in self.skip_downsamplings)

    def forward(self, inputs, plan=None):
        if self.backbone_rgbd is not None:
            return self._forward_single('rgbd', self.backbone_rgbd, inputs['rgbd'], plan)
        rgb, depth = inputs.get('rgb'), inputs.get('depth')
        if self._twin_eval_ok(plan, rgb):
            return self._forward_twin_eval(rgb, depth)
        skips = {}
        bb = self.backbone_rgb if self.backbone_rgb is not None else self.backbone_depth
        dual = self.two and _dual_stream(rgb)
        if dual:
            cur = torch.cuda.current_stream()
            if self._side_stream is None:
                self._side_stream = torch.cuda.Stream()
            side = self._side_stream
            from .parallel import register_stream
            register_stream(cur)
            register_stream(side)
        for i, ds in enumerate(bb.stage_downsamplings):
            if dual:
                side.wait_stream(cur)
                rgb = self.backbone_rgb.forward_stage(i, rgb)
                with torch.cuda.stream(side):
                    depth = self.backbone_depth.forward_stage(i, depth)
                cur.wait_stream(side)
                depth.record_stream(cur)
            else:
                if rgb is not None:
                    rgb = self.backbone_rgb.forward_stage(i, rgb)
                if depth is not None:
                    depth = self.backbone_depth.forward_stage(i, depth)
            if self.two:
                rgb, depth = self.fusion_modules[i](rgb, depth)
            if ds in self.skip_downsamplings:
                skips[str(ds)] = {k: (v if plan is None else (v, i))
                                  for k, v in (('rgb', rgb), ('depth', depth)) if v is not None}
            if plan is not None and i in plan.stages:
                if rgb is not None:
                    rgb = plan.cut(rgb, i, i)
                if depth is not None:
                    depth = plan.cut(depth, i, i)
        last = len(bb.stage_downsamplings) - 1
        outs = {k: (v if plan is None else (v, last))
                for k, v in (('rgb', rgb), ('depth', depth)) if v is not None}
        return outs, skips

    def _twin_eval_ok(self, plan, x=None):
        if not (self.two and plan is None and _fast_eval(self) and twin_launches(x)):
            return False
        r, d = self.backbone_rgb, self.backbone_depth
        if r.compute_dtype == torch.float32 or r.compute_dtype != d.compute_dtype or not Fn.CONV_RS:
            return False
        for i in range(1, 5):
            lr, ld = getattr(r, f'layer{i}'), getattr(d, f'layer{i}')
            if len(lr) != len(ld) or not all(isinstance(m, NonBottleneck1D) for m in list(lr) + list(ld)):
                return False
        return True

    def _forward_twin_eval(self, rgb, depth):
        r, d = self.backbone_rgb, self.backbone_depth
        skips = {}
        for i, ds in enumerate(r.stage_downsamplings):
            if i == 0:
                rgb, depth = r.forward_stage(0, rgb), d.forward_stage(0, depth)
            else:
                if i == 1:
                    rgb, depth = ops.MaxPoolFunction.apply(rgb), ops.MaxPoolFunction.apply(depth)
                rgb, depth = Fn.as_act(rgb, dense=True), Fn.as_act(depth, dense=True)
                for br, bd in zip(getattr(r, f'layer{i}'), getattr(d, f'layer{i}')):
                    rgb, depth = ops.nbt1d_eval_pair(rgb, depth, br._rt, bd._rt)
            rgb, depth = self.fusion_modules[i](rgb, depth)
            if ds in self.skip_downsamplings:
                skips[str(ds)] = {'rgb': rgb, 'depth': depth}
        return {'rgb': rgb, 'depth': depth}, skips

    def _forward_single(self, key, bb, x, plan):
        skips = {}
        for i, ds in enumerate(bb.stage_downsamplings):
            x = bb.forward_stage(i, x)
            if ds in self.skip_downsamplings:
                skips[str(ds)] = {key: x if plan is None else (x, i)}
            if plan is not None and i in plan.stages:
                x = plan.cut(x, i, i)
        last = len(bb.stage_downsamplings) - 1
        return {key: x if plan is None else (x, last)}, skips

    def stage_parameters(self, i):
        ps = []
        for bb in (self.backbone_rgb, self.backbone_depth, self.backbone_rgbd):
            if bb is None:
                continue
            mods = [bb.conv1, bb.bn1] if i == 0 else [getattr(bb, f'layer{i}')]
            for m in mods:
                ps += list(m.parameters())
        if self.two:
            ps += list(self.fusion_modules[i].parameters())
        return ps


class PyramidPoolingModule(nn.Module):

    def __init__(self, cin, cout, input_size, upsampling='bilinear'):
        super().__init__()
        if upsampling not in ('bilinear', 'nearest'):
            raise NotImplementedError(f"upsampling_context_module='{upsampling}'")
        self.upsampling = upsampling
        bins = Spec.PPM_BINS
        self.bins = bins
        self.n_channels_reduction = cin // len(bins)
        self.features = nn.ModuleList([
            nn.Sequential(nn.Identity(), ConvNormAct(cin, self.n_channels_reduction, 1))
            for _ in bins])
        self.final_conv = ConvNormAct(cin + self.n_channels_reduction * len(bins), cout, 1)

    def forward(self, x):
        feats = []
        for b, f in zip(self.bins, self.features):
            feats.append(f[1](ops.AdaptiveAvgPoolFunction.apply(x, b)))
        cat = ops.PPMConcatFunction.apply(x, *feats, self.upsampling)
        return self.final_conv(cat), tuple(feats)


class LearnedUpsampling(nn.Module):

    def __init__(self, c, c_pad=None):
        super().__init__()
        self.conv = nn.Conv2d(c, c, 3, padding=1, groups=c, bias=Spec.DW_UPSAMPLE_BIAS)
        w = torch.tensor([[1., 2., 1.], [2., 4., 2.], [1., 2., 1.]]) / 16.
        with torch.no_grad():
            self.conv.weight.copy_(w.expand(c, 1, 3, 3))
            if self.conv.bias is not None:
                self.conv.bias.zero_()
        self.c, self.c_pad = c, c_pad or c

    def _padded(self):
        w, b = self.conv.weight, self.conv.bias
        if self.c_pad != self.c:
            key = None
            if not torch.is_grad_enabled():
                key = (w._version, w.data_ptr(), None if b is None else (b._version, b.data_ptr()))
                hit = getattr(self, '_pad_cache', None)
                if hit is not None and hit[0] == key:
                    return hit[1], hit[2]
            w = torch.cat([w, w.new_zeros(self.c_pad - self.c, 1, 3, 3)], 0)
            if b is not None:
                b = torch.cat([b, b.new_zeros(self.c_pad - self.c)], 0)
            if key is not None:
                self._pad_cache = (key, w, b)
        return w, b

    def forward(self, x, skip=None, out_f32=False):
        w, b = self._padded()
        return ops.UpsampleDWFunction.apply(x, w, b, skip, out_f32)

    @staticmethod
    def eval_pair(ma, mb, xa, xb, ska, skb):
        (wa, ba), (wb, bb) = ma._padded(), mb._padded()
        xa, xb = Fn.as_act(xa, dense=True), Fn.as_act(xb, dense=True)
        if ska is not None and skb is not None:
            ska, skb = Fn.as_act(ska, dense=True), Fn.as_act(skb, dense=True)
        det = lambda t: None if t is None else t.detach()
        r = Fn.up2x_dw_fwd_pair((xa, xb), (wa.detach().contiguous(), wb.detach().contiguous()),
                                (det(ba), det(bb)), (ska, skb)) if wa.shape == wb.shape else None
        return r if r is not None else (ma(xa, ska), mb(xb, skb))


class PlainUpsampling(nn.Module):

    def __init__(self, mode):
        super().__init__()
        self.mode = mode

    def forward(self, x, skip=None, out_f32=False):
        return ops.PlainUpsampleFunction.apply(x, self.mode, skip, out_f32)


UPSAMPLING_MODES = ('learned-3x3-zeropad', 'nearest', 'bilinear')


def make_upsampling(mode, c, c_pad=None):
    if mode == 'learned-3x3-zeropad':
        return LearnedUpsampling(c, c_pad)
    if mode in ('nearest', 'bilinear'):
        return PlainUpsampling(mode)
    raise NotImplementedError(f"upsampling '{mode}' (built: {', '.join(UPSAMPLING_MODES)})")


def make_plain_conv_rt(conv):
    k = conv.kernel_size[0]
    return ops.MultiConvRT([(conv, 0, 0)], Fn.pad8(conv.out_channels), conv.in_channels, k,
                           conv.padding[0])


def plain_conv(rt, x):
    return ops.MultiConvFunction.apply(x, rt, *rt.params())
```

emsanet_amd/ops.py:

```python
import os

import torch
from torch.autograd import Function
from torch.autograd.function import once_differentiable

from . import _lib
from . import functional as Fn
from ._lib import check
from .functional import ACT_NONE, ACT_RELU
from .parallel import grad_target

TRACE = None
MASK_TRACE = None


GRAD_TRACE = None


def _trace_grad(module, dy):
    if GRAD_TRACE is not None:
        GRAD_TRACE[id(module)] = dy.detach().float().cpu()


def _trace_mask(tag, t):
# ... 1000 lines not shown
                               wino2d_u=self._wino2d_weights()[0])
        if self.wino:
            return Fn.conv_fwd(x, None, self.spec, bias=bias, wino_u=self._u)
        return Fn.conv_fwd(x, wp, self.spec, bias=bias)

    def real_flops(self, x):
        n, _, h, w = x.shape
        return 2.0 * n * h * w * sum(m.weight.numel() for m, _, _ in self.placements)

    def dgrad(self, dy, in_hw):
        Fn.prof_flops(self.real_flops(dy))
        key = self._key_now()
        ent = self._hd.get(dy.dtype)
        if ent is None or ent[0] != key:
            wpd = self.packed_dgrad(dy.dtype)
            ud = None
            if self.wino and dy.dtype == torch.float32:
                s = self.spec
                ud = Fn.pack_wino_packed(wpd, s.cin, s.cout, Fn.wino_rows(s), flip=True)
            ent = (key, wpd, ud)
            self._hd[dy.dtype] = ent
        _, wpd, ud = ent
        if ud is not None and self.wino2d:
            return Fn.conv_dgrad(dy, None, self.spec, in_hw, wino_u=ud,
                                 wino2d_u=self._wino2d_weights()[1])
        if ud is not None:
            return Fn.conv_dgrad(dy, None, self.spec, in_hw, wino_u=ud)
        return Fn.conv_dgrad(dy, wpd, self.spec, in_hw)

    def packed_dgrad(self, dtype=torch.float32):
        s = self.spec
        wp = torch.zeros(s.kh * s.kw * s.cout * s.cin, device=self.placements[0][0].weight.device,
                         dtype=dtype)
        for m, co, ci in self.placements:
            if dtype == torch.float32:
                Fn.pack_weight(self._w4(m).detach(), 'dgrad', s.cout, co, s.cin, ci, out=wp)
            else:
                Fn.pack_weight_t(self._w4(m).detach(), dtype, False, True, s.cout, co, s.cin, ci,
                                 out_dgrad=wp)
        return wp

    def params(self):
        ps = []
        for m, _, _ in self.placements:
            ps.append(m.weight)
            if m.bias is not None:
                ps.append(m.bias)
        return ps


class MultiConvFunction(Function):
    @staticmethod
    def forward(ctx, x, rt, *params):
        x = Fn.as_act(x)
        y = rt.forward(x)
        ctx.rt = rt
        ctx.save_for_backward(x)
        return y

    @staticmethod
    @once_differentiable
    @_traced
    def backward(ctx, dy):
        rt = ctx.rt
        (x,) = ctx.saved_tensors
        dy = Fn.as_act(dy)
        s = rt.spec
        Fn.prof_flops(rt.real_flops(x))
        if GRAD_TRACE is not None:
            for m, co, _ in rt.placements:
                _trace_grad(m, dy[:, co:co + m.weight.shape[0]])
        dwp, db, _ = Fn.conv_wgrad(x, dy, s, rt.has_bias)
        grads = []
        for m, co, ci in rt.placements:
            w4 = rt._w4(m)
            tw = grad_target(m.weight)
            dw = Fn.unpack_wgrad(dwp, w4, s.cout, co, s.cin, ci,
                                 out=tw.view(w4.shape) if tw is not None else None)
            grads.append(tw if tw is not None else dw.reshape(m.weight.shape))
            if m.bias is not None:
                grads.append(db[co:co + m.bias.shape[0]].clone())
        dx = None
        if ctx.needs_input_grad[0]:
            dx = rt.dgrad(dy, x.shape[2:])
        return (dx, None) + tuple(grads)


class StemRT:
    def __init__(self, conv, bn):
        self.conv, self.brt = conv, BNRT(bn)
        self.spec = Fn.StemSpec(conv.in_channels, conv.out_channels)
        self._packs = {}

    def packed(self, dtype=torch.float32):
        w = self.conv.weight
        key = (w._version, w.data_ptr())
        ent = self._packs.get(dtype)
        if ent is None or ent[0] != key:
            ent = (key, Fn.stem_pack_weight(w.detach(), dtype))
            self._packs[dtype] = ent
        return ent[1]


class StemFunction(Function):
    @staticmethod
    def forward(ctx, x_nchw, rt, weight, gamma, beta, bias=None, dtype=torch.float32):
        n, c, h, w = x_nchw.shape
        xp = Fn.stem_pack_input(x_nchw.detach().float(), dtype)
        brt = rt.brt
        b = bias.detach() if bias is not None else None
        wpk = rt.packed(dtype)
        if brt.batch_stats():
            y, stats = Fn.stem_fwd(xp, wpk, rt.spec, n, h, w, want_stats=True, bias=b)
            count = y.shape[0] * y.shape[2] * y.shape[3]
        else:
            y, _ = Fn.stem_fwd(xp, wpk, rt.spec, n, h, w, want_stats=False, bias=b)
            stats, count = None, 0
        scale, shift, mean, invstd = brt.forward_stats(stats, count)
        out, mask = Fn.bn_act(y, scale, shift, None, None, ACT_RELU, want_mask=True)
        _trace_mask('stem', out)
        ctx.rt = rt
        ctx.hw = (n, h, w)
        ctx.saved = (xp, y, mean, invstd, mask)
        ctx.bn_train = brt.batch_stats()
        ctx.has_bias = bias is not None
        return out

    @staticmethod
    @once_differentiable
    @_traced
    def backward(ctx, dout):
        rt = ctx.rt
        xp, y, mean, invstd, mask = ctx.saved
        ctx.saved = None
        n, h, w = ctx.hw
        dout = Fn.as_act(dout, dense=True)
        dy, _, dg, db = Fn.bn_bwd(dout, mask, y, rt.brt.bn.weight.detach(), mean, invstd, None,
                                  ACT_RELU, ctx.bn_train, want_dres=False, **_bn_targets(rt.brt))
        _trace_grad(rt.conv, dy)
        res = Fn.stem_wgrad(xp, dy, rt.spec, n, h, w, rt.conv.weight,
                            out=grad_target(rt.conv.weight), want_bias=ctx.has_bias)
        dw, dbias = res if ctx.has_bias else (res, None)
        return None, None, dw, dg, db, dbias, None


def stem_eval(x_nchw, rt, dtype=torch.float32):
    n, c, h, w = x_nchw.shape
    xp = Fn.stem_pack_input(x_nchw.float(), dtype)
    s, t = rt.brt.folded()
    b = rt.conv.bias.detach() if rt.conv.bias is not None else None
    return Fn.stem_fwd_folded(xp, rt.packed(dtype), rt.spec, n, h, w, s, t, bias=b)


class MaxPoolFunction(Function):
    @staticmethod
    def forward(ctx, x):
        x = Fn.as_act(x, dense=True)
        y, idx = Fn.maxpool_fwd(x)
        ctx.idx, ctx.hw = idx, tuple(x.shape[2:])
        return y

    @staticmethod
    @once_differentiable
    @_traced
    def backward(ctx, dy):
        return Fn.maxpool_bwd(Fn.as_act(dy, dense=True), ctx.idx, ctx.hw)


SE_PAIR = os.environ.get('EMSA_SE_PAIR', '1') != '0'


def _se_params(se):
    f0, f2 = se.fc[0], se.fc[2]
    return [f0.weight, f0.bias, f2.weight, f2.bias]


class SEAddFunction(Function):

    @staticmethod
    def forward(ctx, rgb, depth, w1r, b1r, w2r, b2r, w1d, b1d, w2d, b2d):
        rgb, depth = Fn.as_act(rgb, dense=True), Fn.as_act(depth, dense=True)
        flat = lambda w: w.detach().reshape(w.shape[0], -1)
        if SE_PAIR:
            gr, gd, hr, hd, sr, sd = Fn.se_pair_fwd(
                rgb, depth, (flat(w1r), b1r.detach(), flat(w2r), b2r.detach()),
                (flat(w1d), b1d.detach(), flat(w2d), b2d.detach()))
        else:
            gr, gd = Fn.channel_mean(rgb), Fn.channel_mean(depth)
            hr, sr = Fn.se_mlp_fwd(gr, flat(w1r), b1r.detach(), flat(w2r), b2r.detach())
            hd, sd = Fn.se_mlp_fwd(gd, flat(w1d), b1d.detach(), flat(w2d), b2d.detach())
        _trace_mask('se.rgb', hr)
        _trace_mask('se.depth', hd)
        out = Fn.se_scale_add(rgb, sr, depth, sd)
        ctx.set_materialize_grads(False)
        ctx.save_for_backward(rgb, depth)
        ctx.saved = (gr, gd, hr, sr, hd, sd, flat(w1r), flat(w2r), flat(w1d), flat(w2d))
        ctx.shapes = (w1r.shape, w2r.shape)
        return out, depth[:]

    @staticmethod
    @once_differentiable
    @_traced
    def backward(ctx, dout, ddepth_next):
        rgb, depth = ctx.saved_tensors
        gr, gd, hr, sr, hd, sd, w1r, w2r, w1d, w2d = ctx.saved
        ctx.saved = None
        if dout is None:
            dout = torch.zeros_like(rgb)
        dout = Fn.as_act(dout, dense=True)
        if ddepth_next is not None:
            ddepth_next = Fn.as_act(ddepth_next, dense=True)
            if ddepth_next.dtype != dout.dtype:
                ddepth_next = Fn.cast(ddepth_next, dout.dtype)
        s1, s2 = ctx.shapes
        res = []
        for x, g, h, s, w1, w2, extra in ((rgb, gr, hr, sr, w1r, w2r, None),
                                          (depth, gd, hd, sd, w1d, w2d, ddepth_next)):
            ds = Fn.se_scale_bwd_reduce(dout, x)
            dgap, dw1, db1, dw2, db2 = Fn.se_mlp_bwd(g, w1, w2, h, s, ds)
            dx = Fn.se_scale_bwd_apply(dout, s, dgap, extra)
            res.append((dx, dw1.reshape(s1), db1, dw2.reshape(s2), db2))
        (dr, a1, a2, a3, a4), (dd, e1, e2, e3, e4) = res
        return dr, dd, a1, a2, a3, a4, e1, e2, e3, e4


class UpsampleDWFunction(Function):

    @staticmethod
    def forward(ctx, x, wdw, bias, skip, out_f32=False):
        x = Fn.as_act(x, dense=True)
        if skip is not None:
            skip = Fn.as_act(skip, dense=True)
        w = wdw.detach().contiguous()
        y = Fn.up2x_dw_fwd(x, w, bias.detach() if bias is not None else None, skip,
                           out_f32=out_f32 and x.dtype != torch.float32)
        ctx.save_for_backward(x, w)
        ctx.has = (bias is not None, skip is not None)
        ctx.wshape = wdw.shape
        return y

    @staticmethod
    @once_differentiable
    @_traced
    def backward(ctx, dy):
        x, w = ctx.saved_tensors
        dy = Fn.as_act(dy, dense=True)
        dx, dw, db = Fn.up2x_dw_bwd(dy, x, w, need_dx=ctx.needs_input_grad[0])
        has_bias, has_skip = ctx.has
        dskip = None
        if has_skip:
            dskip = dy if dy.dtype == x.dtype else Fn.cast(dy, x.dtype)
        return dx, dw.reshape(ctx.wshape), (db if has_bias else None), dskip, None


class PlainUpsampleFunction(Function):

    @staticmethod
    def forward(ctx, x, mode, skip, out_f32=False):
        if mode not in ('bilinear', 'nearest'):
            raise NotImplementedError(f"upsampling '{mode}'")
        x = Fn.as_act(x, dense=True)
        ctx.mode, ctx.x_dtype, ctx.hw = mode, x.dtype, tuple(x.shape[2:])
        if out_f32 and x.dtype != torch.float32:
            x = Fn.cast(x, torch.float32)
        n, c, h, w = x.shape
        y = Fn.act_empty(n, c, 2 * h, 2 * w, x.device, dtype=x.dtype)
        (Fn.bilinear_fwd if mode == 'bilinear' else Fn.nearest_fwd)(x, y)
        ctx.has_skip = skip is not None
        if skip is not None:
            skip = Fn.as_act(skip, dense=True)
            y = Fn.add(y, skip if skip.dtype == y.dtype else Fn.cast(skip, y.dtype))
        return y

    @staticmethod
    @once_differentiable
    @_traced
    def backward(ctx, dy):
        dy = Fn.as_act(dy, dense=True)
        dx = None
        if ctx.needs_input_grad[0]:
            dx = (Fn.bilinear_bwd if ctx.mode == 'bilinear' else Fn.nearest_bwd)(dy, ctx.hw)
            if dx.dtype != ctx.x_dtype:
                dx = Fn.cast(dx, ctx.x_dtype)
        dskip = None
        if ctx.has_skip:
            dskip = dy if dy.dtype == ctx.x_dtype else Fn.cast(dy, ctx.x_dtype)
        return dx, None, dskip, None


class AdaptiveAvgPoolFunction(Function):
    @staticmethod
    def forward(ctx, x, bins):
        x = Fn.as_act(x, dense=True)
        ctx.bins, ctx.shape = bins, tuple(x.shape)
        return Fn.adaptive_avgpool_fwd(x, bins)

    @staticmethod
    @once_differentiable
    @_traced
    def backward(ctx, dy):
        n, c, h, w = ctx.shape
        dy = Fn.as_act(dy, dense=True)
        dx = Fn.act_empty(n, c, h, w, dy.device, dtype=dy.dtype)
        Fn.adaptive_avgpool_bwd(dy, dx, ctx.bins, accumulate=False)
        return dx, None

# ... 94 lines not shown
```

include/emsanet_hip.h:

```cpp
#ifndef EMSANET_HIP_H
#define EMSANET_HIP_H

#include <stdint.h>

#ifdef __cplusplus
extern "C" {
#endif

#define EMSA_OK 0
#define EMSA_E_SHAPE (-1)
#define EMSA_E_ARG (-2)
#define EMSA_E_LAUNCH (-3)

#define EMSA_ACT_NONE 0
#define EMSA_ACT_RELU 1

#define EMSA_DT_F32 0
#define EMSA_DT_BF16 1
#define EMSA_DT_F16 2

const char* emsa_arch(void);
int emsa_version(void);
int emsa_set_batch_invariant(int on);

// ... 371 lines not shown
                               uint8_t* stack, void* stream);

int emsa_conv_stats_rows_t(int32_t dtype, const EmsaConvGeom* g);
int emsa_conv_igemm_t(int32_t dtype, const EmsaConvGeom* g, const void* in, const void* w,
                      void* out, const float* bias, float* stats, const float* scale,
                      const float* shift, const void* residual, int32_t ld_res,
                      const void* mask_src, int32_t ld_mask, int32_t act, void* stream);
int64_t emsa_conv_igemm_splitk_ws_bytes_t(int32_t dtype, const EmsaConvGeom* g);
int emsa_conv_igemm_splitk_t(int32_t dtype, const EmsaConvGeom* g, const void* in, const void* w,
                             void* out, const float* bias, const float* scale, const float* shift,
                             const void* residual, int32_t ld_res, int32_t act, float* ws,
                             void* stream);
int emsa_conv_igemm_pair_t(int32_t dtype, const EmsaConvGeom* g, const void* in0, const void* in1,
                           const void* w0, const void* w1, void* out0, void* out1,
                           const float* bias0, const float* bias1, const float* scale0,
                           const float* scale1, const float* shift0, const float* shift1,
                           const void* residual0, const void* residual1, int32_t ld_res,
                           int32_t act, float* ws0, float* ws1, void* stream);
int emsa_conv_igemm_bnb_t(int32_t dtype, const EmsaConvGeom* g, const void* dy, const void* w,
                          void* out, const void* residual, int32_t ld_res, const void* t,
                          int32_t ld_t, const float* bn_scale, const float* bn_shift,
                          const float* bn_mean, const float* bn_invstd, float* partial,
                          int32_t rows_alloc, void* stream);
int emsa_bn_bwd_apply_rows_t(int32_t dtype, const void* g, const void* x, const float* gamma,
                             const float* save_mean, const float* save_invstd, float* partial,
                             int32_t rows, int32_t n_img, int64_t hw, int32_t c, int32_t train,
                             void* dx, float* dgamma, float* dbeta, void* stream);
int64_t emsa_conv_wgrad_ws_bytes_t(int32_t dtype, const EmsaConvGeom* g);
int emsa_conv_wgrad_t(int32_t dtype, const EmsaConvGeom* g, const void* in, const void* dout,
                      float* dw, float* dbias, float* ws, void* stream);
int64_t emsa_conv_wgrad_multi_ws_bytes(int32_t dtype, int32_t n_jobs, const EmsaConvGeom* geoms);
int emsa_conv_wgrad_multi_t(int32_t dtype, int32_t n_jobs, const EmsaConvGeom* geoms,
                            const void* const* in, const void* const* dout, float* const* dw,
                            float* const* dbias, float* ws, void* stream);
int emsa_pack_weight_t(int32_t dtype, const float* w, void* wp_fwd, void* wp_dgrad, int32_t cout,
                       int32_t cin, int32_t kh, int32_t kw, int32_t cout_total, int32_t cout_off,
                       int32_t cin_total, int32_t cin_off, void* stream);
int emsa_stem_pack_weight_t(int32_t dtype, const float* w, void* wp, int32_t cout, int32_t cin,
                            void* stream);

int emsa_nbt_half_block_supported(int32_t dtype, int32_t c, int32_t w);
int emsa_nbt_half_block_t(int32_t dtype, int32_t n_sets, int32_t n_img, int32_t h, int32_t w,
                          int32_t c, const void* const* in, int32_t ld_in, const void* const* wfa,
                          const float* const* bias_a, const void* const* wfb,
                          const float* const* bias_b, const float* const* scale,
                          const float* const* shift, const void* const* residual, int32_t ld_res,
                          void* const* out, int32_t ld_out, int32_t act, void* stream);
int emsa_conv_rs_set_cu_budget(int32_t cus);
int emsa_conv1d_rs_supported(int32_t dtype, const EmsaConvGeom* g);
int emsa_conv1d_rs_stats_rows(int32_t dtype, const EmsaConvGeom* g);
int emsa_conv1d_rs_t(int32_t dtype, const EmsaConvGeom* g, const void* in, const void* wfrag,
                     void* out, const float* bias, float* stats, const float* scale,
                     const float* shift, const void* residual, int32_t ld_res,
                     const void* mask_src, int32_t ld_mask, int32_t act, void* stream);
int emsa_conv1d_rs_pair_t(int32_t dtype, const EmsaConvGeom* g, const void* in0, const void* in1,
                          const void* wfrag0, const void* wfrag1, void* out0, void* out1,
                          const float* bias0, const float* bias1, const float* scale0,
                          const float* scale1, const float* shift0, const float* shift1,
                          const void* residual0, const void* residual1, int32_t ld_res,
                          int32_t act, void* stream);
int emsa_conv1d_rs_bnb_t(int32_t dtype, const EmsaConvGeom* g, const void* dy, const void* wfrag,
                         void* out, const void* residual, int32_t ld_res, const void* t,
                         int32_t ld_t, const float* bn_scale, const float* bn_shift,
                         const float* bn_mean, const float* bn_invstd, float* partial,
                         int32_t rows_alloc, void* stream);
int emsa_pack_weight_frag_t(int32_t dtype, const float* w_oihw, void* wf_fwd, void* wf_dgrad,
                            int32_t cout, int32_t cin, void* stream);

int emsa_conv1d_rs_inbn_t(int32_t dtype, const EmsaConvGeom* g, const void* in, const void* wfrag,
                          void* out, const float* bias, float* stats, const float* in_scale,
                          const float* in_shift, int32_t act, void* stream);
int emsa_conv_wgrad_inbn_t(int32_t dtype, const EmsaConvGeom* g, const void* in, const void* dout,
                           float* dw, float* dbias, float* ws, const float* in_scale,
                           const float* in_shift, void* stream);
int emsa_conv_wgrad_multi_inbn_t(int32_t dtype, int32_t n_jobs, const EmsaConvGeom* geoms,
                                 const void* const* in, const void* const* dout, float* const* dw,
                                 float* const* dbias, float* ws, const float* const* in_scale,
                                 const float* const* in_shift, void* stream);
int emsa_bn_bwd_reduce_aff_t(int32_t dtype, const void* dy, const void* x, const float* save_mean,
                             const float* save_invstd, const float* mask_scale,
                             const float* mask_shift, int32_t n_img, int64_t hw, int32_t c,
                             float* partial, void* stream);
int emsa_bn_bwd_apply_aff_t(int32_t dtype, const void* dy, const void* x, const float* gamma,
                            const float* save_mean, const float* save_invstd,
                            const float* mask_scale, const float* mask_shift, float* partial,
                            int32_t rows_alloc, int32_t n_img, int64_t hw, int32_t c, void* dx,
                            float* dgamma, float* dbeta, void* stream);

int emsa_bn_act_fwd_t(int32_t dtype, const void* x, void* y, const float* scale, const float*
    shift, const float* drop, const void* residual, int32_t n_img, int64_t hw, int32_t c,
    int32_t act, uint64_t* mask_bits, void* stream);
int emsa_bn_bwd_reduce_t(int32_t dtype, const void* dy, const void* y, const uint64_t*
    mask_bits, const void* x, const float* save_mean, const float* save_invstd, const float*
    drop, int32_t n_img, int64_t hw, int32_t c, int32_t act, float* partial, void* stream);
int emsa_bn_bwd_apply_t(int32_t dtype, const void* dy, const void* y, const uint64_t* mask_bits,
    const void* x, const float* gamma, const float* save_mean, const float* save_invstd, const
    float* drop, float* partial, int32_t rows_alloc, int32_t n_img, int64_t hw, int32_t c,
    int32_t act, int32_t train, void* dx, void* dres, float* dgamma, float* dbeta, void*
    stream);
int emsa_maxpool3x3s2_fwd_t(int32_t dtype, const void* x, void* y, int8_t* idx, int32_t n,
    int32_t h, int32_t w, int32_t c, void* stream);
int emsa_maxpool3x3s2_bwd_t(int32_t dtype, const void* dy, const int8_t* idx, void* dx, int32_t
    n, int32_t h, int32_t w, int32_t c, void* stream);
int emsa_se_scale_add_fwd_t(int32_t dtype, const void* a, const float* sa, const void* b, const
    float* sb, void* out, int32_t n, int64_t hw, int32_t c, void* stream);
int emsa_se_scale_bwd_apply_t(int32_t dtype, const void* dout, const float* s, const float*
    dgap, const void* dx_extra, void* dx, int32_t n, int64_t hw, int32_t c, void* stream);
int emsa_up2x_dw3x3_fwd_t(int32_t dtype, int32_t out_f32, const void* x, const float* wdw, const
    float* bias, const void* skip, void* y, int32_t n, int32_t h, int32_t w, int32_t c, void*
    stream);
int emsa_up2x_dw3x3_fwd_pair_t(int32_t dtype, const void* x0, const void* x1, const float* wdw0,
                               const float* wdw1, const float* bias0, const float* bias1,
                               const void* skip0, const void* skip1, void* y0, void* y1, int32_t n,
                               int32_t h, int32_t w, int32_t c, void* stream);
int emsa_up2x_dw3x3_bwd_data_t(int32_t dtype, int32_t out_f32, const void* dy, const float* wdw,
    void* dx, int32_t n, int32_t h, int32_t w, int32_t c, void* stream);
int emsa_up2x_dw3x3_bwd_weight_t(int32_t dtype, int32_t out_f32, const void* dy, const void* x,
    float* dw, float* db, int32_t n, int32_t h, int32_t w, int32_t c, void* stream);
int emsa_up2x_dw3x3_bwd_t(int32_t dtype, int32_t out_f32, const void* dy, const void* x, const
    float* wdw, void* dx, float* dw, float* db, int32_t n, int32_t h, int32_t w, int32_t c, void*
    stream);
int emsa_adaptive_avgpool_fwd_t(int32_t dtype, const void* x, void* y, int32_t n, int32_t h,
    int32_t w, int32_t c, int32_t bins, void* stream);
int emsa_adaptive_avgpool_bwd_t(int32_t dtype, const void* dy, void* dx, int32_t n, int32_t h,
    int32_t w, int32_t c, int32_t bins, int32_t accumulate, void* stream);
int emsa_bilinear_fwd_t(int32_t dtype, const void* x, void* y, int32_t n, int32_t ih, int32_t
    iw, int32_t oh, int32_t ow, int32_t c, int32_t ld_y, void* stream);
int emsa_bilinear_bwd_t(int32_t dtype, const void* dy, float* dx, int32_t n, int32_t ih, int32_t
    iw, int32_t oh, int32_t ow, int32_t c, int32_t ld_dy, void* stream);
int emsa_add_t(int32_t dtype, const void* a, const void* b, void* out, int64_t n, void* stream);
int emsa_nearest_fwd_t(int32_t dtype, const void* x, void* y, int32_t n, int32_t ih, int32_t iw,
    int32_t oh, int32_t ow, int32_t c, int32_t ld_y, void* stream);
int emsa_nearest_bwd_t(int32_t dtype, const void* dy, float* dx, int32_t n, int32_t ih, int32_t iw,
    int32_t oh, int32_t ow, int32_t c, int32_t ld_dy, void* stream);
int emsa_head_act_fwd_t(int32_t dtype, int32_t out_f32, const void* x, void* y, int64_t pixels,
    int32_t c, int32_t n_sig, int32_t n_tanh, int32_t norm_off, int32_t n_norm, void* stream);
int emsa_head_act_bwd_gather_t(int32_t dtype, const float* g0, int32_t ld0, int32_t c0, const float* g1,
                               int32_t ld1, int32_t c1, const float* g2, int32_t ld2, int32_t c2,
                               const float* y, const void* x, void* dx, int64_t pixels, int32_t c,
                               int32_t n_sig, int32_t n_tanh, int32_t norm_off, int32_t n_norm,
                               void* stream);
int emsa_head_act_bwd_t(int32_t dtype, int32_t out_f32, const void* dy, const void* y, const
    void* x, void* dx, int64_t pixels, int32_t c, int32_t n_sig, int32_t n_tanh, int32_t
    norm_off, int32_t n_norm, void* stream);
int emsa_stem_pack_input_t(int32_t dtype, const float* x, void* xp, int32_t n, int32_t c,
    int32_t h, int32_t w, void* stream);
int emsa_se_pair_fwd_t(int32_t dtype, const void* xa, const void* xb, float* ws, const float* w1a,
                       const float* b1a, const float* w2a, const float* b2a, const float* w1b,
                       const float* b1b, const float* w2b, const float* b2b, float* gap,
                       float* hid, float* s, int32_t n, int64_t hw, int32_t c, int32_t cr,
                       void* stream);
int emsa_channel_mean_t(int32_t dtype, const void* x, float* gap, float* ws, int32_t n, int64_t
    hw, int32_t c, void* stream);
int emsa_se_scale_bwd_reduce_t(int32_t dtype, const void* dout, const void* x, float* ds, float*
    ws, int32_t n, int64_t hw, int32_t c, void* stream);
int emsa_cast_channels(int32_t src_dtype, const void* x, int32_t ld_x, int32_t dst_dtype, void*
    y, int32_t ld_y, int64_t pixels, int32_t c, void* stream);
int emsa_to_nhwc_t(int32_t dtype, const void* x, void* y, int32_t n, int32_t c, int32_t h,
                   int32_t w, int64_t s_n, int64_t s_c, int64_t s_h, int64_t s_w, void* stream);

int emsa_memset_async(void* dst, int32_t value, int64_t bytes, void* stream);
int emsa_graph_count_nodes(void* graph, int32_t* n_nodes, int32_t* n_memset, int32_t* n_kernel);
int emsa_graph_replace_memsets(void* graph, int32_t* replaced);

int emsa_prof_enable(int32_t every);
int emsa_prof_next_flops(double flops);
int emsa_prof_reset(void);
int emsa_prof_seen(int32_t cls);
const char* emsa_prof_name(int32_t cls);
int emsa_prof_read(int32_t cls, double* total_ms, double* total_flops, int32_t* launches);
int emsa_prof_read_bytes(int32_t cls, double* total_bytes);

#ifdef __cplusplus
}
#endif
#endif
```

Baseline: 329.5 images/s.

## Fuse stem BN-ReLU, SE fusion and maxpool into dedicated stage kernels

Adds a fused stem stage for both modalities. The forward pass folds BN affine, ReLU, SE squeeze, the SE pair MLP, the SE-add fusion and the 3x3/2 maxpool into a few kernels that store int8 argmax indices. The backward pass unpools by quads, runs the BN/SE gradient reductions in one pass and applies dx in another, so no full-resolution intermediate activations are materialized and several elementwise launches are dropped. The cost is significant new kernel code specialized for C=64 f32, and the possibility that the wiring into the model is only partly shown.

```diff
diff --git a/emsanet_amd/_lib.py b/emsanet_amd/_lib.py
--- a/emsanet_amd/_lib.py
+++ b/emsanet_amd/_lib.py
@@ -239,6 +239,13 @@
     'emsa_channel_mean_t': (c_int, [c_int32, _P, _P, _P, c_int32, c_int64, c_int32, _P]),
     'emsa_se_pair_fwd_t': (c_int, [c_int32] + [_P] * 14 + [c_int32, c_int64, c_int32, c_int32, _P]),
     'emsa_se_scale_bwd_reduce_t': (c_int, [c_int32, _P, _P, _P, _P, c_int32, c_int64, c_int32, _P]),
+    'emsa_se_pair_mlp_fwd': (c_int, [_P] * 12 + [c_int32, c_int64, c_int32, c_int32, _P]),
+    'emsa_stem_stage_squeeze': (c_int, [_P] * 7 + [c_int32, c_int64, c_int32, _P]),
+    'emsa_stem_stage_fwd': (c_int, [_P] * 12 + [c_int32] * 4 + [_P]),
+    'emsa_stem_stage_bwd_splits': (c_int, [c_int32, c_int32]),
+    'emsa_stem_stage_bwd_reduce': (c_int, [_P] * 17 + [c_int32] * 4 + [_P]),
+    'emsa_stem_stage_bwd_finalize': (c_int, [_P] * 9 + [c_int32, c_int64, c_int32, _P]),
+    'emsa_stem_stage_bwd_apply': (c_int, [_P] * 26 + [c_int32] * 4 + [_P]),
     'emsa_cast_channels': (c_int, [c_int32, _P, c_int32, c_int32, _P, c_int32, c_int64, c_int32, _P]),
     'emsa_conv_stats_rows_t': (c_int, [c_int32, _GP]),
     'emsa_conv_igemm_t': (c_int, [c_int32, _GP, _P, _P, _P, _P, _P, _P, _P, _P, c_int32, _P, c_int32,
diff --git a/emsanet_amd/csrc/bn_math.h b/emsanet_amd/csrc/bn_math.h
--- /dev/null
+++ b/emsanet_amd/csrc/bn_math.h
@@ -0,0 +1,21 @@
+#pragma once
+#include <hip/hip_runtime.h>
+
+__device__ __forceinline__ float bn_mul(float a, float b) {
+#pragma clang fp contract(off)
+  return a * b;
+}
+__device__ __forceinline__ float bn_add(float a, float b) {
+#pragma clang fp contract(off)
+  return a + b;
+}
+__device__ __forceinline__ float bn_affine(float x, float sc, float sh) { return __builtin_fmaf(x, sc, sh); }
+__device__ __forceinline__ float bn_acc_xhat(float acc, float g, float x, float mu, float is) {
+  return __builtin_fmaf(bn_mul(g, bn_add(x, -mu)), is, acc);
+}
+__device__ __forceinline__ float bn_dx_train(float g, float x, float mu, float is, float gi, float db,
+                                             float dg, float inv_count) {
+  const float xh = bn_mul(bn_add(x, -mu), is);
+  const float t = __builtin_fmaf(-db, inv_count, g);
+  return bn_mul(gi, __builtin_fmaf(-bn_mul(xh, dg), inv_count, t));
+}
diff --git a/emsanet_amd/csrc/pointwise.hip b/emsanet_amd/csrc/pointwise.hip
--- a/emsanet_amd/csrc/pointwise.hip
+++ b/emsanet_amd/csrc/pointwise.hip
@@ -4,6 +4,7 @@
 
 #include <atomic>
 #include "common.h"
+#include "bn_math.h"
 
 namespace {
 
@@ -275,25 +276,6 @@
     shift[i] = beta[i] - rm[i] * sc;
     if (invstd) invstd[i] = is;
   }
-}
-
-__device__ __forceinline__ float bn_mul(float a, float b) {
-#pragma clang fp contract(off)
-  return a * b;
-}
-__device__ __forceinline__ float bn_add(float a, float b) {
-#pragma clang fp contract(off)
-  return a + b;
-}
-__device__ __forceinline__ float bn_affine(float x, float sc, float sh) { return __builtin_fmaf(x, sc, sh); }
-__device__ __forceinline__ float bn_acc_xhat(float acc, float g, float x, float mu, float is) {
-  return __builtin_fmaf(bn_mul(g, bn_add(x, -mu)), is, acc);
-}
-__device__ __forceinline__ float bn_dx_train(float g, float x, float mu, float is, float gi, float db,
-                                             float dg, float inv_count) {
-  const float xh = bn_mul(bn_add(x, -mu), is);
-  const float t = __builtin_fmaf(-db, inv_count, g);
-  return bn_mul(gi, __builtin_fmaf(-bn_mul(xh, dg), inv_count, t));
 }
 
 template <typename T> struct VecIO {
@@ -2925,6 +2907,20 @@
                                                       s, n, (long)hw, c, cr, (hipStream_t)stream));
   return EMSA_E_ARG;
 }
+extern "C" int emsa_se_pair_mlp_fwd(const float* ws, const float* w1a, const float* b1a,
+                                    const float* w2a, const float* b2a, const float* w1b,
+                                    const float* b1b, const float* w2b, const float* b2b,
+                                    float* gap, float* hid, float* s, int32_t n, int64_t hw,
+                                    int32_t c, int32_t cr, void* stream) {
+  if (!ws || !w1a || !b1a || !w2a || !b2a || !w1b || !b1b || !w2b || !b2b || !gap || !hid || !s)
+    return EMSA_E_ARG;
+  if (n < 1 || hw < 1 || c < 1 || cr < 1) return EMSA_E_SHAPE;
+  hipLaunchKernelGGL(se_mlp_pair_fwd_kernel, dim3(2 * n), dim3(256),
+                     (size_t)(c + cr) * sizeof(float), (hipStream_t)stream, ws,
+                     channel_splits((long)hw, n), 1.0f / (float)hw, w1a, b1a, w2a, b2a, w1b, b1b, w2b,
+                     b2b, gap, hid, s, n, c, cr);
+  return emsa_launch_status();
+}
 extern "C" int emsa_se_mlp_bwd(const float* gap, const float* w1, const float* w2,
                                const float* hid, const float* s, const float* ds, float* dgap,
                                float* dw1, float* db1, float* dw2, float* db2, int32_t n,
diff --git a/emsanet_amd/csrc/stem_stage.hip b/emsanet_amd/csrc/stem_stage.hip
--- /dev/null
+++ b/emsanet_amd/csrc/stem_stage.hip
@@ -0,0 +1,529 @@
+#include <cstdlib>
+
+#include "common.h"
+#include "bn_math.h"
+
+namespace {
+
+constexpr int kThreads = 256;
+constexpr int kC = 64;
+constexpr int kCvn = kC / 4;
+constexpr int kLanes = kThreads / kCvn;
+constexpr int kSums = 12;
+constexpr int kMaxBlocks = 256 * 8;
+enum { Q_DS = 0, Q_A0 = 1, Q_A1 = 2, Q_M0 = 3, Q_M1 = 4, Q_DEPTH = 5, Q_D0 = 10, Q_D1 = 11 };
+
+__device__ __forceinline__ void ld4v(const float* p, float (&v)[4]) {
+  const float4 f = emsa_ld4(p);
+  v[0] = f.x; v[1] = f.y; v[2] = f.z; v[3] = f.w;
+}
+__device__ __forceinline__ void cvt4(const float4& f, float (&v)[4]) {
+  v[0] = f.x; v[1] = f.y; v[2] = f.z; v[3] = f.w;
+}
+
+struct StemAffine {
+  const float* scale[2];
+  const float* shift[2];
+};
+struct StemStats {
+  const float* mean[2];
+  const float* invstd[2];
+};
+
+__global__ __launch_bounds__(kThreads) void stem_squeeze_kernel(
+    const float* __restrict__ y_rgb, const float* __restrict__ y_depth, const StemAffine aff,
+    float* __restrict__ ws, long hw, int splits, int nblk) {
+  __shared__ __attribute__((aligned(16))) float cred[kLanes * kC];
+  const bool second = (int)blockIdx.x >= nblk;
+  const int blk = second ? blockIdx.x - nblk : blockIdx.x;
+  const float* __restrict__ y = second ? y_depth : y_rgb;
+  const int img = blk / splits, sp = blk % splits;
+  const long chunk = (hw + splits - 1) / splits;
+  const long p0 = img * hw + sp * chunk, p1 = min(img * hw + (sp + 1) * chunk, (img + 1) * hw);
+  const int cv = threadIdx.x % kCvn, rl = threadIdx.x / kCvn;
+  float sc[4], sh[4], acc[4] = {0.f, 0.f, 0.f, 0.f};
+  ld4v((second ? aff.scale[1] : aff.scale[0]) + cv * 4, sc);
+  ld4v((second ? aff.shift[1] : aff.shift[0]) + cv * 4, sh);
+  auto term = [&](const float4& r) {
+    float v[4];
+    cvt4(r, v);
+#pragma unroll
+    for (int k = 0; k < 4; ++k) acc[k] += fmaxf(bn_affine(v[k], sc[k], sh[k]), 0.f);
+  };
+  long p = p0 + rl;
+  for (; p + 3 * kLanes < p1; p += 4 * kLanes) {
+    float4 r[4];
+#pragma unroll
+    for (int u = 0; u < 4; ++u) r[u] = emsa_ld4(y + ((p + u * kLanes) * kCvn + cv) * 4);
+#pragma unroll
+    for (int u = 0; u < 4; ++u) term(r[u]);
+  }
+  for (; p < p1; p += kLanes) term(emsa_ld4(y + (p * kCvn + cv) * 4));
+#pragma unroll
+  for (int k = 0; k < 4; ++k) cred[rl * kC + cv * 4 + k] = acc[k];
+  __syncthreads();
+  for (int ch = threadIdx.x; ch < kC; ch += kThreads) {
+    float t = 0.f;
+    for (int k = 0; k < kLanes; ++k) t += cred[k * kC + ch];
+    ws[(long)blockIdx.x * kC + ch] = t;
+  }
+}
+
+template <typename I>
+__global__ __launch_bounds__(kThreads) void stem_pool_fwd_kernel(
+    const float* __restrict__ y_rgb, const float* __restrict__ y_depth, const StemAffine aff,
+    const float* __restrict__ s_rgb, const float* __restrict__ s_depth, float* __restrict__ pf,
+    int8_t* __restrict__ idx_f, float* __restrict__ pd, int8_t* __restrict__ idx_d, int n, int h,
+    int w) {
+  const int oh_n = (h + 1) / 2, ow_n = (w + 1) / 2;
+  const I total = (I)n * oh_n * ow_n * kCvn;
+  const int c4 = threadIdx.x % kCvn;
+  float scr[4], shr[4], scd[4], shd[4];
+  ld4v(aff.scale[0] + c4 * 4, scr);
+  ld4v(aff.shift[0] + c4 * 4, shr);
+  ld4v(aff.scale[1] + c4 * 4, scd);
+  ld4v(aff.shift[1] + c4 * 4, shd);
+  for (I i = blockIdx.x * (I)kThreads + threadIdx.x; i < total; i += (I)gridDim.x * kThreads) {
+    I r = i / (I)kCvn;
+    const int ow = (int)(r % (I)ow_n); r /= (I)ow_n;
+    const int oh = (int)(r % (I)oh_n);
+    const int img = (int)(r / (I)oh_n);
+    float4 tr[9], td[9];
+#pragma unroll
+    for (int kh = 0; kh < 3; ++kh)
+#pragma unroll
+      for (int kw = 0; kw < 3; ++kw) {
+        const int ih = min(max(oh * 2 - 1 + kh, 0), h - 1), iw = min(max(ow * 2 - 1 + kw, 0), w - 1);
+        const size_t o = (size_t)(((((I)img * h + ih) * w + iw) * kCvn + c4) * 4);
+        tr[kh * 3 + kw] = emsa_ld4(y_rgb + o);
+        td[kh * 3 + kw] = emsa_ld4(y_depth + o);
+      }
+    float sr[4], sd[4];
+    ld4v(s_rgb + ((size_t)img * kCvn + c4) * 4, sr);
+    ld4v(s_depth + ((size_t)img * kCvn + c4) * 4, sd);
+    float bf[4], bd[4];
+    int kf[4] = {0, 0, 0, 0}, kd[4] = {0, 0, 0, 0};
+#pragma unroll
+    for (int k = 0; k < 4; ++k) bf[k] = bd[k] = -INFINITY;
+    bool first = true;
+#pragma unroll
+    for (int kh = 0; kh < 3; ++kh)
+#pragma unroll
+      for (int kw = 0; kw < 3; ++kw) {
+        const int ih = oh * 2 - 1 + kh, iw = ow * 2 - 1 + kw, t = kh * 3 + kw;
+        const bool in = ih >= 0 && ih < h && iw >= 0 && iw < w;
+        float vr[4], vd[4];
+        cvt4(tr[t], vr);
+        cvt4(td[t], vd);
+#pragma unroll
+        for (int k = 0; k < 4; ++k) {
+          const float ar = fmaxf(bn_affine(vr[k], scr[k], shr[k]), 0.f);
+          const float ad = fmaxf(bn_affine(vd[k], scd[k], shd[k]), 0.f);
+          const float f = __builtin_fmaf(ar, sr[k], bn_mul(ad, sd[k]));
+          if (in && (first || f > bf[k])) { bf[k] = f; kf[k] = t; }
+          if (in && (first || ad > bd[k])) { bd[k] = ad; kd[k] = t; }
+        }
+        first = first && !in;
+      }
+    emsa_st4(pf + (size_t)i * 4, make_float4(bf[0], bf[1], bf[2], bf[3]));
+    emsa_st4(pd + (size_t)i * 4, make_float4(bd[0], bd[1], bd[2], bd[3]));
+    *reinterpret_cast<char4*>(idx_f + (size_t)i * 4) = make_char4(kf[0], kf[1], kf[2], kf[3]);
+    *reinterpret_cast<char4*>(idx_d + (size_t)i * 4) = make_char4(kd[0], kd[1], kd[2], kd[3]);
+  }
+}
+
+struct QuadIn {
+  float4 gf[4], gd[4];
+  uint32_t kf[4], kd[4];
+  float4 yr[4], yd[4];
+};
+
+template <typename I>
+__device__ __forceinline__ void quad_issue(QuadIn& q, const float* __restrict__ gf,
+                                           const int8_t* __restrict__ idx_f,
+                                           const float* __restrict__ gd,
+                                           const int8_t* __restrict__ idx_d,
+                                           const float* __restrict__ y_rgb,
+                                           const float* __restrict__ y_depth, int img, int qh, int qw,
+                                           int c4, int h, int w, int oh_n, int ow_n) {
+#pragma unroll
+  for (int dh = 0; dh < 2; ++dh)
+#pragma unroll
+    for (int dw = 0; dw < 2; ++dw) {
+      const int oh = min(qh + dh, oh_n - 1), ow = min(qw + dw, ow_n - 1);
+      const size_t o = (size_t)(((((I)img * oh_n + oh) * ow_n + ow) * kCvn + c4) * 4);
+      q.gf[dh * 2 + dw] = emsa_ld4(gf + o);
+      q.gd[dh * 2 + dw] = emsa_ld4(gd + o);
+      q.kf[dh * 2 + dw] = *reinterpret_cast<const uint32_t*>(idx_f + o);
+      q.kd[dh * 2 + dw] = *reinterpret_cast<const uint32_t*>(idx_d + o);
+    }
+#pragma unroll
+  for (int a = 0; a < 2; ++a)
+#pragma unroll
+    for (int b = 0; b < 2; ++b) {
+      const int ih = min(2 * qh + a, h - 1), iw = min(2 * qw + b, w - 1);
+      const size_t o = (size_t)(((((I)img * h + ih) * w + iw) * kCvn + c4) * 4);
+      q.yr[a * 2 + b] = emsa_ld4(y_rgb + o);
+      q.yd[a * 2 + b] = emsa_ld4(y_depth + o);
+    }
+}
+
+__device__ __forceinline__ void quad_unpool(const QuadIn& q, int qh, int qw, int oh_n, int ow_n,
+                                            float (&dout)[4][4], float (&dd)[4][4]) {
+#pragma unroll
+  for (int p = 0; p < 4; ++p)
+#pragma unroll
+    for (int k = 0; k < 4; ++k) dout[p][k] = dd[p][k] = 0.f;
+#pragma unroll
+  for (int dh = 0; dh < 2; ++dh)
+#pragma unroll
+    for (int dw = 0; dw < 2; ++dw) {
+      const bool valid = qh + dh < oh_n && qw + dw < ow_n;
+      float g[4], e[4];
+      cvt4(q.gf[dh * 2 + dw], g);
+      cvt4(q.gd[dh * 2 + dw], e);
+      const uint32_t rf = q.kf[dh * 2 + dw], rd = q.kd[dh * 2 + dw];
+#pragma unroll
+      for (int a = 0; a < 2; ++a) {
+        const int kh = a - 2 * dh + 1;
+        if (kh < 0 || kh > 2) continue;
+#pragma unroll
+        for (int b = 0; b < 2; ++b) {
+          const int kw = b - 2 * dw + 1;
+          if (kw < 0 || kw > 2) continue;
+          const uint32_t t = (uint32_t)(kh * 3 + kw);
+#pragma unroll
+          for (int k = 0; k < 4; ++k) {
+            dout[a * 2 + b][k] += (valid && ((rf >> (8 * k)) & 0xFFu) == t) ? g[k] : 0.f;
+            dd[a * 2 + b][k] += (valid && ((rd >> (8 * k)) & 0xFFu) == t) ? e[k] : 0.f;
+          }
+        }
+      }
+    }
+}
+
+__device__ __forceinline__ void quad_range(int oh_n, int ow_n, int splits, int sp, int& q0, int& q1) {
+  const int nq = oh_n * ow_n, chunk = (nq + splits - 1) / splits;
+  q0 = sp * chunk;
+  q1 = min(nq, q0 + chunk);
+}
+
+template <typename I>
+__global__ __launch_bounds__(kThreads, 2) void stem_bwd_reduce_kernel(
+    const float* __restrict__ gf, const int8_t* __restrict__ idx_f, const float* __restrict__ gd,
+    const int8_t* __restrict__ idx_d, const float* __restrict__ y_rgb,
+    const float* __restrict__ y_depth, const StemAffine aff, const StemStats st,
+    float* __restrict__ ws, int h, int w, int splits) {
+  __shared__ __attribute__((aligned(16))) float cred[kSums * kLanes * kC];
+  const int oh_n = (h + 1) / 2, ow_n = (w + 1) / 2;
+  const int img = blockIdx.x / splits, sp = blockIdx.x % splits;
+  int q0, q1;
+  quad_range(oh_n, ow_n, splits, sp, q0, q1);
+  const int c4 = threadIdx.x % kCvn, rl = threadIdx.x / kCvn;
+  float sc[2][4], sh[2][4], mu[2][4], is[2][4];
+#pragma unroll
+  for (int m = 0; m < 2; ++m) {
+    ld4v(aff.scale[m] + c4 * 4, sc[m]);
+    ld4v(aff.shift[m] + c4 * 4, sh[m]);
+    ld4v(st.mean[m] + c4 * 4, mu[m]);
+    ld4v(st.invstd[m] + c4 * 4, is[m]);
+  }
+  float acc[kSums][4];
+#pragma unroll
+  for (int s = 0; s < kSums; ++s)
+#pragma unroll
+    for (int k = 0; k < 4; ++k) acc[s][k] = 0.f;
+  for (int qi = q0 + rl; qi < q1; qi += kLanes) {
+    const int qh = qi / ow_n, qw = qi - qh * ow_n;
+    QuadIn q;
+    quad_issue<I>(q, gf, idx_f, gd, idx_d, y_rgb, y_depth, img, qh, qw, c4, h, w, oh_n, ow_n);
+    float dout[4][4], dd[4][4];
+    quad_unpool(q, qh, qw, oh_n, ow_n, dout, dd);
+#pragma unroll
+    for (int p = 0; p < 4; ++p) {
+      const bool pv = 2 * qh + (p >> 1) < h && 2 * qw + (p & 1) < w;
+#pragma unroll
+      for (int m = 0; m < 2; ++m) {
+        float y[4];
+        cvt4(m ? q.yd[p] : q.yr[p], y);
+#pragma unroll
+        for (int k = 0; k < 4; ++k) {
+          const float z = bn_affine(y[k], sc[m][k], sh[m][k]);
+          const bool on = pv && z > 0.f;
+          const float g = on ? dout[p][k] : 0.f;
+          const float xh = bn_mul(bn_add(y[k], -mu[m][k]), is[m][k]);
+          acc[m * Q_DEPTH + Q_DS][k] = __builtin_fmaf(dout[p][k], fmaxf(z, 0.f), acc[m * Q_DEPTH + Q_DS][k]);
+          acc[m * Q_DEPTH + Q_A0][k] = bn_add(acc[m * Q_DEPTH + Q_A0][k], g);
+          acc[m * Q_DEPTH + Q_A1][k] = bn_acc_xhat(acc[m * Q_DEPTH + Q_A1][k], g, y[k], mu[m][k], is[m][k]);
+          acc[m * Q_DEPTH + Q_M0][k] += on ? 1.f : 0.f;
+          acc[m * Q_DEPTH + Q_M1][k] += on ? xh : 0.f;
+          if (m == 1) {
+            const float e = on ? dd[p][k] : 0.f;
+            acc[Q_D0][k] = bn_add(acc[Q_D0][k], e);
+            acc[Q_D1][k] = bn_acc_xhat(acc[Q_D1][k], e, y[k], mu[m][k], is[m][k]);
+          }
+        }
+      }
+    }
+  }
+#pragma unroll
+  for (int s = 0; s < kSums; ++s)
+#pragma unroll
+    for (int k = 0; k < 4; ++k) cred[(s * kLanes + rl) * kC + c4 * 4 + k] = acc[s][k];
+  __syncthreads();
+  for (int o = threadIdx.x; o < kSums * kC; o += kThreads) {
+    const int s = o / kC, ch = o % kC;
+    float t = 0.f;
+    for (int k = 0; k < kLanes; ++k) t += cred[(s * kLanes + k) * kC + ch];
+    ws[((long)blockIdx.x * kSums + s) * kC + ch] = t;
+  }
+}
+
+__global__ void stem_bwd_merge_kernel(const float* __restrict__ ws, int splits, int n,
+                                      double* __restrict__ sums, float* __restrict__ ds) {
+  const int img = blockIdx.x, o = blockIdx.y * blockDim.x + threadIdx.x;
+  if (o >= kSums * kC) return;
+  double a = 0.0;
+#pragma unroll 4
+  for (int sp = 0; sp < splits; ++sp) a += (double)ws[((long)img * splits + sp) * kSums * kC + o];
+  sums[(long)img * kSums * kC + o] = a;
+  const int s = o / kC, ch = o % kC;
+  if (s == Q_DS) ds[(long)img * kC + ch] = (float)a;
+  if (s == Q_DEPTH + Q_DS) ds[((long)n + img) * kC + ch] = (float)a;
+}
+
+struct StemGradOut {
+  float* dgamma[2];
+  float* dbeta[2];
+};
+__global__ void stem_bwd_finalize_kernel(const double* __restrict__ sums,
+                                         const float* __restrict__ s_rgb,
+                                         const float* __restrict__ s_depth,
+                                         const float* __restrict__ dgap_rgb,
+                                         const float* __restrict__ dgap_depth, const StemGradOut out,
+                                         int n, double inv_hw) {
+  const int m = threadIdx.x / kC, ch = threadIdx.x % kC;
+  const float* __restrict__ s = m ? s_depth : s_rgb;
+  const float* __restrict__ dgap = m ? dgap_depth : dgap_rgb;
+  double db = 0.0, dg = 0.0;
+  for (int img = 0; img < n; ++img) {
+    const double* __restrict__ r = sums + ((long)img * kSums + m * Q_DEPTH) * kC + ch;
+    const double sv = (double)s[(long)img * kC + ch], dv = (double)dgap[(long)img * kC + ch] * inv_hw;
+    db += sv * r[Q_A0 * kC] + dv * r[Q_M0 * kC];
+    dg += sv * r[Q_A1 * kC] + dv * r[Q_M1 * kC];
+    if (m == 1) {
+      db += sums[((long)img * kSums + Q_D0) * kC + ch];
+      dg += sums[((long)img * kSums + Q_D1) * kC + ch];
+    }
+  }
+  (m ? out.dbeta[1] : out.dbeta[0])[ch] = (float)db;
+  (m ? out.dgamma[1] : out.dgamma[0])[ch] = (float)dg;
+}
+
+struct StemApplyVec {
+  const float* gamma[2];
+  const float* s[2];
+  const float* dgap[2];
+  const float* dgamma[2];
+  const float* dbeta[2];
+};
+template <typename I>
+__global__ __launch_bounds__(kThreads, 2) void stem_bwd_apply_kernel(
+    const float* __restrict__ gf, const int8_t* __restrict__ idx_f, const float* __restrict__ gd,
+    const int8_t* __restrict__ idx_d, const float* __restrict__ y_rgb,
+    const float* __restrict__ y_depth, const StemAffine aff, const StemStats st,
+    const StemApplyVec v, float* __restrict__ dy_rgb, float* __restrict__ dy_depth, int h, int w,
+    int splits, float inv_hw, float inv_count) {
+  const int oh_n = (h + 1) / 2, ow_n = (w + 1) / 2;
+  const int img = blockIdx.x / splits, sp = blockIdx.x % splits;
+  int q0, q1;
+  quad_range(oh_n, ow_n, splits, sp, q0, q1);
+  const int c4 = threadIdx.x % kCvn, rl = threadIdx.x / kCvn;
+  float sc[2][4], sh[2][4], mu[2][4], is[2][4], gi[2][4], db[2][4], dg[2][4], sv[2][4], dv[2][4];
+#pragma unroll
+  for (int m = 0; m < 2; ++m) {
+    float ga[4], dgp[4];
+    ld4v(aff.scale[m] + c4 * 4, sc[m]);
+    ld4v(aff.shift[m] + c4 * 4, sh[m]);
+    ld4v(st.mean[m] + c4 * 4, mu[m]);
+    ld4v(st.invstd[m] + c4 * 4, is[m]);
+    ld4v(v.gamma[m] + c4 * 4, ga);
+    ld4v(v.dbeta[m] + c4 * 4, db[m]);
+    ld4v(v.dgamma[m] + c4 * 4, dg[m]);
+    ld4v(v.s[m] + ((size_t)img * kCvn + c4) * 4, sv[m]);
+    ld4v(v.dgap[m] + ((size_t)img * kCvn + c4) * 4, dgp);
+#pragma unroll
+    for (int k = 0; k < 4; ++k) {
+      gi[m][k] = bn_mul(ga[k], is[m][k]);
+      dv[m][k] = bn_mul(dgp[k], inv_hw);
+    }
+  }
+  for (int qi = q0 + rl; qi < q1; qi += kLanes) {
+    const int qh = qi / ow_n, qw = qi - qh * ow_n;
+    QuadIn q;
+    quad_issue<I>(q, gf, idx_f, gd, idx_d, y_rgb, y_depth, img, qh, qw, c4, h, w, oh_n, ow_n);
+    float dout[4][4], dd[4][4];
+    quad_unpool(q, qh, qw, oh_n, ow_n, dout, dd);
+#pragma unroll
+    for (int p = 0; p < 4; ++p) {
+      const int ih = 2 * qh + (p >> 1), iw = 2 * qw + (p & 1);
+      if (ih >= h || iw >= w) continue;
+      const size_t o = (size_t)(((((I)img * h + ih) * w + iw) * kCvn + c4) * 4);
+#pragma unroll
+      for (int m = 0; m < 2; ++m) {
+        float y[4], r[4];
+        cvt4(m ? q.yd[p] : q.yr[p], y);
+#pragma unroll
+        for (int k = 0; k < 4; ++k) {
+          float da = __builtin_fmaf(dout[p][k], sv[m][k], dv[m][k]);
+          if (m == 1) da = bn_add(da, dd[p][k]);
+          const float dz = bn_affine(y[k], sc[m][k], sh[m][k]) > 0.f ? da : 0.f;
+          r[k] = bn_dx_train(dz, y[k], mu[m][k], is[m][k], gi[m][k], db[m][k], dg[m][k], inv_count);
+        }
+        emsa_st4((m ? dy_depth : dy_rgb) + o, make_float4(r[0], r[1], r[2], r[3]));
+      }
+    }
+  }
+}
+
+bool idx32_ok(long max_elements) {
+  static const bool on = [] {
+    const char* e = getenv("EMSA_IDX32");
+    return !e || atoi(e) != 0;
+  }();
+  return on && max_elements > 0 && max_elements < (1L << 31);
+}
+
+bool shape_ok(int n, long h, long w, int c) {
+  return c == kC && n >= 1 && h >= 1 && w >= 1 && h < (1 << 24) && w < (1 << 24) &&
+         (long)n * ((h + 1) / 2) * ((w + 1) / 2) < (1L << 31) / kCvn;
+}
+
+int bwd_splits(int h, int w) {
+  const long nq = (long)((h + 1) / 2) * ((w + 1) / 2);
+  long s = (nq + 255) / 256;
+  return (int)(s < 1 ? 1 : s > 64 ? 64 : s);
+}
+
+}
+
+extern "C" int emsa_stem_stage_squeeze(const float* y_rgb, const float* y_depth,
+                                       const float* scale_rgb, const float* shift_rgb,
+                                       const float* scale_depth, const float* shift_depth,
+                                       float* ws, int32_t n, int64_t hw, int32_t c, void* stream) {
+  if (!y_rgb || !y_depth || !scale_rgb || !shift_rgb || !scale_depth || !shift_depth || !ws)
+    return EMSA_E_ARG;
+  if (c != kC || n < 1 || hw < 1) return EMSA_E_SHAPE;
+  const int splits = emsa_channel_ws_floats(n, hw, c) / (n * c);
+  if (splits < 1 || (long)2 * n * splits >= (1L << 31)) return EMSA_E_SHAPE;
+  const StemAffine aff = {{scale_rgb, scale_depth}, {shift_rgb, shift_depth}};
+  hipLaunchKernelGGL(stem_squeeze_kernel, dim3(2 * n * splits), dim3(kThreads), 0,
+                     (hipStream_t)stream, y_rgb, y_depth, aff, ws, (long)hw, splits, n * splits);
+  return emsa_launch_status();
+}
+
+extern "C" int emsa_stem_stage_fwd(const float* y_rgb, const float* y_depth, const float* scale_rgb,
+                                   const float* shift_rgb, const float* scale_depth,
+                                   const float* shift_depth, const float* s_rgb,
+                                   const float* s_depth, float* pf, int8_t* idx_f, float* pd,
+                                   int8_t* idx_d, int32_t n, int32_t h, int32_t w, int32_t c,
+                                   void* stream) {
+  if (!y_rgb || !y_depth || !scale_rgb || !shift_rgb || !scale_depth || !shift_depth || !s_rgb ||
+      !s_depth || !pf || !idx_f || !pd || !idx_d)
+    return EMSA_E_ARG;
+  if (!shape_ok(n, h, w, c)) return EMSA_E_SHAPE;
+  const StemAffine aff = {{scale_rgb, scale_depth}, {shift_rgb, shift_depth}};
+  const long total = (long)n * ((h + 1) / 2) * ((w + 1) / 2) * kCvn;
+  long blocks = (total + kThreads - 1) / kThreads;
+  if (blocks > kMaxBlocks) blocks = kMaxBlocks;
+  const dim3 grid((int)blocks), block(kThreads);
+  if (idx32_ok((long)n * h * w * c))
+    hipLaunchKernelGGL(stem_pool_fwd_kernel<uint32_t>, grid, block, 0, (hipStream_t)stream, y_rgb,
+                       y_depth, aff, s_rgb, s_depth, pf, idx_f, pd, idx_d, n, h, w);
+  else
+    hipLaunchKernelGGL(stem_pool_fwd_kernel<long>, grid, block, 0, (hipStream_t)stream, y_rgb,
+                       y_depth, aff, s_rgb, s_depth, pf, idx_f, pd, idx_d, n, h, w);
+  return emsa_launch_status();
+}
+
+extern "C" int emsa_stem_stage_bwd_splits(int32_t h, int32_t w) {
+  return h >= 1 && w >= 1 ? bwd_splits(h, w) : EMSA_E_SHAPE;
+}
+
+extern "C" int emsa_stem_stage_bwd_reduce(const float* gf, const int8_t* idx_f, const float* gd,
+                                          const int8_t* idx_d, const float* y_rgb,
+                                          const float* y_depth, const float* scale_rgb,
+                                          const float* shift_rgb, const float* scale_depth,
+                                          const float* shift_depth, const float* mean_rgb,
+                                          const float* invstd_rgb, const float* mean_depth,
+                                          const float* invstd_depth, float* ws, double* sums,
+                                          float* ds, int32_t n, int32_t h, int32_t w, int32_t c,
+                                          void* stream) {
+  if (!gf || !idx_f || !gd || !idx_d || !y_rgb || !y_depth || !scale_rgb || !shift_rgb ||
+      !scale_depth || !shift_depth || !mean_rgb || !invstd_rgb || !mean_depth || !invstd_depth ||
+      !ws || !sums || !ds)
+    return EMSA_E_ARG;
+  if (!shape_ok(n, h, w, c)) return EMSA_E_SHAPE;
+  const int splits = bwd_splits(h, w);
+  const StemAffine aff = {{scale_rgb, scale_depth}, {shift_rgb, shift_depth}};
+  const StemStats st = {{mean_rgb, mean_depth}, {invstd_rgb, invstd_depth}};
+  hipStream_t s = (hipStream_t)stream;
+  if (idx32_ok((long)n * h * w * c))
+    hipLaunchKernelGGL(stem_bwd_reduce_kernel<uint32_t>, dim3(n * splits), dim3(kThreads), 0, s, gf,
+                       idx_f, gd, idx_d, y_rgb, y_depth, aff, st, ws, h, w, splits);
+  else
+    hipLaunchKernelGGL(stem_bwd_reduce_kernel<long>, dim3(n * splits), dim3(kThreads), 0, s, gf,
+                       idx_f, gd, idx_d, y_rgb, y_depth, aff, st, ws, h, w, splits);
+  hipLaunchKernelGGL(stem_bwd_merge_kernel, dim3(n, (kSums * kC + 255) / 256), dim3(256), 0, s, ws,
+                     splits, n, sums, ds);
+  return emsa_launch_status();
+}
+
+extern "C" int emsa_stem_stage_bwd_finalize(const double* sums, const float* s_rgb,
+                                            const float* s_depth, const float* dgap_rgb,
+                                            const float* dgap_depth, float* dgamma_rgb,
+                                            float* dbeta_rgb, float* dgamma_depth,
+                                            float* dbeta_depth, int32_t n, int64_t hw, int32_t c,
+                                            void* stream) {
+  if (!sums || !s_rgb || !s_depth || !dgap_rgb || !dgap_depth || !dgamma_rgb || !dbeta_rgb ||
+      !dgamma_depth || !dbeta_depth)
+    return EMSA_E_ARG;
+  if (c != kC || n < 1 || hw < 1) return EMSA_E_SHAPE;
+  const StemGradOut out = {{dgamma_rgb, dgamma_depth}, {dbeta_rgb, dbeta_depth}};
+  hipLaunchKernelGGL(stem_bwd_finalize_kernel, dim3(1), dim3(2 * kC), 0, (hipStream_t)stream, sums,
+                     s_rgb, s_depth, dgap_rgb, dgap_depth, out, n, 1.0 / (double)hw);
+  return emsa_launch_status();
+}
+
+extern "C" int emsa_stem_stage_bwd_apply(
+    const float* gf, const int8_t* idx_f, const float* gd, const int8_t* idx_d, const float* y_rgb,
+    const float* y_depth, const float* scale_rgb, const float* shift_rgb, const float* scale_depth,
+    const float* shift_depth, const float* mean_rgb, const float* invstd_rgb,
+    const float* mean_depth, const float* invstd_depth, const float* gamma_rgb,
+    const float* gamma_depth, const float* s_rgb, const float* s_depth, const float* dgap_rgb,
+    const float* dgap_depth, const float* dgamma_rgb, const float* dbeta_rgb,
+    const float* dgamma_depth, const float* dbeta_depth, float* dy_rgb, float* dy_depth, int32_t n,
+    int32_t h, int32_t w, int32_t c, void* stream) {
+  if (!gf || !idx_f || !gd || !idx_d || !y_rgb || !y_depth || !scale_rgb || !shift_rgb ||
+      !scale_depth || !shift_depth || !mean_rgb || !invstd_rgb || !mean_depth || !invstd_depth ||
+      !gamma_rgb || !gamma_depth || !s_rgb || !s_depth || !dgap_rgb || !dgap_depth || !dgamma_rgb ||
+      !dbeta_rgb || !dgamma_depth || !dbeta_depth || !dy_rgb || !dy_depth)
+    return EMSA_E_ARG;
+  if (!shape_ok(n, h, w, c)) return EMSA_E_SHAPE;
+  const int splits = bwd_splits(h, w);
+  const StemAffine aff = {{scale_rgb, scale_depth}, {shift_rgb, shift_depth}};
+  const StemStats st = {{mean_rgb, mean_depth}, {invstd_rgb, invstd_depth}};
+  const StemApplyVec v = {{gamma_rgb, gamma_depth}, {s_rgb, s_depth}, {dgap_rgb, dgap_depth},
+                          {dgamma_rgb, dgamma_depth}, {dbeta_rgb, dbeta_depth}};
+  const float inv_hw = 1.0f / (float)((long)h * w), inv_count = 1.0f / (float)((long)n * h * w);
+  hipStream_t s = (hipStream_t)stream;
+  if (idx32_ok((long)n * h * w * c))
+    hipLaunchKernelGGL(stem_bwd_apply_kernel<uint32_t>, dim3(n * splits), dim3(kThreads), 0, s, gf,
+                       idx_f, gd, idx_d, y_rgb, y_depth, aff, st, v, dy_rgb, dy_depth, h, w, splits,
+                       inv_hw, inv_count);
+  else
+    hipLaunchKernelGGL(stem_bwd_apply_kernel<long>, dim3(n * splits), dim3(kThreads), 0, s, gf,
+                       idx_f, gd, idx_d, y_rgb, y_depth, aff, st, v, dy_rgb, dy_depth, h, w, splits,
+                       inv_hw, inv_count);
+  return emsa_launch_status();
+}
diff --git a/emsanet_amd/functional.py b/emsanet_amd/functional.py
--- a/emsanet_amd/functional.py
+++ b/emsanet_amd/functional.py
@@ -1166,6 +1166,116 @@
     return dx
 
 
+_STEM_FUSE_ENV = os.environ.get('EMSA_STEM_FUSE')
+_STEM_FUSE_MIN_BYTES = int(float(os.environ.get('EMSA_STEM_FUSE_MIN_MB', '24')) * (1 << 20))
+STEM_FUSE = None
+
+
+STEM_FUSE_FALLBACKS = 0
+
+
+def _stem_fuse_fell_back():
+    global STEM_FUSE_FALLBACKS
+    STEM_FUSE_FALLBACKS += 1
+
+
+def stem_fuse_forced():
+    if STEM_FUSE is not None:
+        return bool(STEM_FUSE)
+    if _STEM_FUSE_ENV is not None:
+        return _STEM_FUSE_ENV != '0'
+    return None
+
+
+def stem_fuse_big_enough(x_nchw, c=64):
+    n, _, h, w = x_nchw.shape
+    return n * c * ((h + 1) // 2) * ((w + 1) // 2) * 4 >= _STEM_FUSE_MIN_BYTES
+
+
+def _stem_pair_check(y_rgb, y_depth):
+    n, c, h, w = y_rgb.shape
+    assert y_depth.shape == y_rgb.shape and y_rgb.dtype == y_depth.dtype == torch.float32
+    assert ld_of(y_rgb) == c and ld_of(y_depth) == c
+    return n, c, h, w
+
+
+def stem_stage_se(y_rgb, y_depth, aff_rgb, aff_depth, wa, wb):
+    n, c, h, w = _stem_pair_check(y_rgb, y_depth)
+    cr = wa[0].shape[0]
+    dev = y_rgb.device
+    L = _lib.lib()
+    gap, hid, s = _empty((2, n, c), dev), _empty((2, n, cr), dev), _empty((2, n, c), dev)
+    ws = _empty((2 * L.emsa_channel_ws_floats(n, h * w, c),), dev)
+    check(L.emsa_stem_stage_squeeze(_p(y_rgb), _p(y_depth), _p(aff_rgb[0]), _p(aff_rgb[1]),
+                                    _p(aff_depth[0]), _p(aff_depth[1]), _p(ws), n, h * w, c,
+                                    _stream()), 'emsa_stem_stage_squeeze')
+    check(L.emsa_se_pair_mlp_fwd(_p(ws), _p(wa[0]), _p(wa[1]), _p(wa[2]), _p(wa[3]), _p(wb[0]),
+                                 _p(wb[1]), _p(wb[2]), _p(wb[3]), _p(gap), _p(hid), _p(s), n, h * w,
+                                 c, cr, _stream()), 'emsa_se_pair_mlp_fwd')
+    return gap[0], gap[1], hid[0], hid[1], s[0], s[1]
+
+
+def stem_stage_fwd(y_rgb, y_depth, aff_rgb, aff_depth, s_rgb, s_depth):
+    n, c, h, w = _stem_pair_check(y_rgb, y_depth)
+    oh, ow = (h + 1) // 2, (w + 1) // 2
+    dev = y_rgb.device
+    pf, pd = act_empty(n, c, oh, ow, dev), act_empty(n, c, oh, ow, dev)
+    idx = _empty((2, n, oh, ow, c), dev, torch.int8)
+    check(_lib.lib().emsa_stem_stage_fwd(_p(y_rgb), _p(y_depth), _p(aff_rgb[0]), _p(aff_rgb[1]),
+                                         _p(aff_depth[0]), _p(aff_depth[1]), _p(s_rgb), _p(s_depth),
+                                         _p(pf), _p(idx[0]), _p(pd), _p(idx[1]), n, h, w, c,
+                                         _stream()), 'emsa_stem_stage_fwd')
+    return pf, idx[0], pd, idx[1]
+
+
+def stem_stage_bwd_reduce(gf, idx_f, gd, idx_d, y_rgb, y_depth, aff_rgb, aff_depth, st_rgb, st_depth):
+    n, c, h, w = _stem_pair_check(y_rgb, y_depth)
+    assert gf.dtype == gd.dtype == torch.float32 and ld_of(gf) == c and ld_of(gd) == c
+    assert tuple(gf.shape) == tuple(gd.shape) == (n, c, (h + 1) // 2, (w + 1) // 2)
+    dev = y_rgb.device
+    L = _lib.lib()
+    splits = L.emsa_stem_stage_bwd_splits(h, w)
+    ws = _empty((n, splits, 12, c), dev)
+    sums = _empty((n, 12, c), dev, torch.float64)
+    ds = _empty((2, n, c), dev)
+    check(L.emsa_stem_stage_bwd_reduce(_p(gf), _p(idx_f), _p(gd), _p(idx_d), _p(y_rgb), _p(y_depth),
+                                       _p(aff_rgb[0]), _p(aff_rgb[1]), _p(aff_depth[0]),
+                                       _p(aff_depth[1]), _p(st_rgb[0]), _p(st_rgb[1]),
+                                       _p(st_depth[0]), _p(st_depth[1]), _p(ws), _p(sums), _p(ds), n,
+                                       h, w, c, _stream()), 'emsa_stem_stage_bwd_reduce')
+    return sums, ds[0], ds[1]
+
+
+def stem_stage_bwd_finalize(sums, hw, s_rgb, s_depth, dgap_rgb, dgap_depth, out_rgb=None,
+                            out_depth=None):
+    n, c = s_rgb.shape
+    res = []
+    for out in (out_rgb, out_depth):
+        if out is None or out[0] is None or out[1] is None:
+            buf = _empty((2, c), s_rgb.device)
+            out = (buf[0], buf[1])
+        res += [out[0], out[1]]
+    check(_lib.lib().emsa_stem_stage_bwd_finalize(_p(sums), _p(s_rgb), _p(s_depth), _p(dgap_rgb),
+                                                  _p(dgap_depth), _p(res[0]), _p(res[1]), _p(res[2]),
+                                                  _p(res[3]), n, hw, c, _stream()),
+          'emsa_stem_stage_bwd_finalize')
+    return tuple(res)
+
+
+def stem_stage_bwd_apply(gf, idx_f, gd, idx_d, y_rgb, y_depth, aff_rgb, aff_depth, st_rgb, st_depth,
+                         gamma_rgb, gamma_depth, s_rgb, s_depth, dgap_rgb, dgap_depth, dgb):
+    n, c, h, w = _stem_pair_check(y_rgb, y_depth)
+    dev = y_rgb.device
+    dy_rgb, dy_depth = act_empty(n, c, h, w, dev), act_empty(n, c, h, w, dev)
+    check(_lib.lib().emsa_stem_stage_bwd_apply(
+        _p(gf), _p(idx_f), _p(gd), _p(idx_d), _p(y_rgb), _p(y_depth), _p(aff_rgb[0]), _p(aff_rgb[1]),
+        _p(aff_depth[0]), _p(aff_depth[1]), _p(st_rgb[0]), _p(st_rgb[1]), _p(st_depth[0]),
+        _p(st_depth[1]), _p(gamma_rgb), _p(gamma_depth), _p(s_rgb), _p(s_depth), _p(dgap_rgb),
+        _p(dgap_depth), _p(dgb[0]), _p(dgb[1]), _p(dgb[2]), _p(dgb[3]), _p(dy_rgb), _p(dy_depth), n,
+        h, w, c, _stream()), 'emsa_stem_stage_bwd_apply')
+    return dy_rgb, dy_depth
+
+
 def _two(name, feat, out_f32, *args):
     code = dt(feat)
     L = _lib.lib()
diff --git a/emsanet_amd/nn.py b/emsanet_amd/nn.py
--- a/emsanet_amd/nn.py
+++ b/emsanet_amd/nn.py
@@ -178,15 +178,19 @@
         self._stem = ops.StemRT(self.conv1, self.bn1)
         self.compute_dtype = torch.float32
 
-    def forward_stage(self, i, x):
+    def forward_stage(self, i, x, pooled=False):
         if i == 0:
             if _fast_eval(self):
                 return ops.stem_eval(x, self._stem, self.compute_dtype)
             return ops.StemFunction.apply(x, self._stem, self.conv1.weight, self.bn1.weight,
                                           self.bn1.bias, self.conv1.bias, self.compute_dtype)
-        if i == 1:
+        if i == 1 and not pooled:
             x = ops.MaxPoolFunction.apply(x)
         return getattr(self, f'layer{i}')(x)
+
+    def stem_conv(self, x):
+        return ops.StemConvFunction.apply(x, self._stem, self.conv1.weight, self.conv1.bias,
+                                          self.compute_dtype)
 
 
 class SqueezeAndExcitation(nn.Module):
@@ -284,6 +288,7 @@
         self.skips_n_channels = tuple(ch[d] for d in self.skip_downsamplings)
 
     def forward(self, inputs, plan=None):
+        fused0 = self._stem_stage_fused(plan, inputs.get('rgb'))
         if self.backbone_rgbd is not None:
             return self._forward_single('rgbd', self.backbone_rgbd, inputs['rgbd'], plan)
         rgb, depth = inputs.get('rgb'), inputs.get('depth')
@@ -301,18 +306,21 @@
             register_stream(cur)
             register_stream(side)
         for i, ds in enumerate(bb.stage_downsamplings):
+            if i == 0 and fused0:
+                rgb, depth = self._forward_stem_stage(rgb, depth, dual and (cur, side))
+                continue
             if dual:
                 side.wait_stream(cur)
-                rgb = self.backbone_rgb.forward_stage(i, rgb)
+                rgb = self.backbone_rgb.forward_stage(i, rgb, pooled=fused0)
                 with torch.cuda.stream(side):
-                    depth = self.backbone_depth.forward_stage(i, depth)
+                    depth = self.backbone_depth.forward_stage(i, depth, pooled=fused0)
                 cur.wait_stream(side)
                 depth.record_stream(cur)
             else:
                 if rgb is not None:
-                    rgb = self.backbone_rgb.forward_stage(i, rgb)
+                    rgb = self.backbone_rgb.forward_stage(i, rgb, pooled=fused0)
                 if depth is not None:
-                    depth = self.backbone_depth.forward_stage(i, depth)
+                    depth = self.backbone_depth.forward_stage(i, depth, pooled=fused0)
             if self.two:
                 rgb, depth = self.fusion_modules[i](rgb, depth)
             if ds in self.skip_downsamplings:
@@ -327,6 +335,40 @@
         outs = {k: (v if plan is None else (v, last))
                 for k, v in (('rgb', rgb), ('depth', depth)) if v is not None}
         return outs, skips
+
+    def _stem_stage_fused(self, plan, x=None):
+        forced = Fn.stem_fuse_forced()
+        if forced is False:
+            return False
+        r, d = self.backbone_rgb, self.backbone_depth
+        ok = self.two and all(
+            bb.training and bb._stem.brt.batch_stats() and bb.compute_dtype == torch.float32 and
+            bb.conv1.out_channels == 64 for bb in (r, d)) and \
+            2 not in self.skip_downsamplings and (plan is None or 0 not in plan.stages)
+        if forced and not ok:
+            Fn._stem_fuse_fell_back()
+        return bool(ok and (forced or (x is not None and Fn.stem_fuse_big_enough(x))))
+
+    def _forward_stem_stage(self, rgb, depth, streams):
+        r, d = self.backbone_rgb, self.backbone_depth
+        if streams:
+            cur, side = streams
+            side.wait_stream(cur)
+            y_rgb, st_rgb = r.stem_conv(rgb)
+            with torch.cuda.stream(side):
+                y_depth, st_depth = d.stem_conv(depth)
+            cur.wait_stream(side)
+            y_depth.record_stream(cur)
+            st_depth.record_stream(cur)
+        else:
+            (y_rgb, st_rgb), (y_depth, st_depth) = r.stem_conv(rgb), d.stem_conv(depth)
+        f = self.fusion_modules[0]
+        pf, pd = ops.StemStageFunction.apply(
+            y_rgb, st_rgb, y_depth, st_depth, r._stem, d._stem, r.bn1.weight, r.bn1.bias,
+            d.bn1.weight, d.bn1.bias, *ops._se_params(f.se_rgb), *ops._se_params(f.se_depth))
+        if streams:
+            pd.record_stream(side)
+        return pf, pd
 
     def _twin_eval_ok(self, plan, x=None):
         if not (self.two and plan is None and _fast_eval(self) and twin_launches(x)):
diff --git a/emsanet_amd/ops.py b/emsanet_amd/ops.py
--- a/emsanet_amd/ops.py
+++ b/emsanet_amd/ops.py
@@ -1176,6 +1176,100 @@
     return Fn.stem_fwd_folded(xp, rt.packed(dtype), rt.spec, n, h, w, s, t, bias=b)
 
 
+class StemConvFunction(Function):
+
+    @staticmethod
+    def forward(ctx, x_nchw, rt, weight, bias=None, dtype=torch.float32):
+        n, c, h, w = x_nchw.shape
+        xp = Fn.stem_pack_input(x_nchw.detach().float(), dtype)
+        b = bias.detach() if bias is not None else None
+        y, stats = Fn.stem_fwd(xp, rt.packed(dtype), rt.spec, n, h, w, want_stats=True, bias=b)
+        ctx.rt, ctx.hw, ctx.xp, ctx.has_bias = rt, (n, h, w), xp, bias is not None
+        ctx.mark_non_differentiable(stats)
+        ctx.set_materialize_grads(False)
+        return y, stats
+
+    @staticmethod
+    @once_differentiable
+    @_traced
+    def backward(ctx, dy, _dstats):
+        rt, xp = ctx.rt, ctx.xp
+        ctx.xp = None
+        n, h, w = ctx.hw
+        dy = Fn.as_act(dy, dense=True)
+        _trace_grad(rt.conv, dy)
+        res = Fn.stem_wgrad(xp, dy, rt.spec, n, h, w, rt.conv.weight,
+                            out=grad_target(rt.conv.weight), want_bias=ctx.has_bias)
+        dw, dbias = res if ctx.has_bias else (res, None)
+        return None, None, dw, dbias, None
+
+
+class StemStageFunction(Function):
+
+    @staticmethod
+    def forward(ctx, y_rgb, stats_rgb, y_depth, stats_depth, rt_rgb, rt_depth, gamma_r, beta_r,
+                gamma_d, beta_d, w1r, b1r, w2r, b2r, w1d, b1d, w2d, b2d):
+        y_rgb, y_depth = Fn.as_act(y_rgb, dense=True), Fn.as_act(y_depth, dense=True)
+        n, c, h, w = y_rgb.shape
+        aff, st = [], []
+        for rt, stats in ((rt_rgb, stats_rgb), (rt_depth, stats_depth)):
+            scale, shift, mean, invstd = rt.brt.forward_stats(stats, n * h * w)
+            aff.append((scale, shift))
+            st.append((mean, invstd))
+        if MASK_TRACE is not None:
+            for y, (scale, shift) in zip((y_rgb, y_depth), aff):
+                _trace_mask('stem', Fn.bn_act(y, scale, shift, None, None, ACT_RELU))
+        flat = lambda t: t.detach().reshape(t.shape[0], -1)
+        gr, gd, hr, hd, sr, sd = Fn.stem_stage_se(
+            y_rgb, y_depth, aff[0], aff[1], (flat(w1r), b1r.detach(), flat(w2r), b2r.detach()),
+            (flat(w1d), b1d.detach(), flat(w2d), b2d.detach()))
+        _trace_mask('se.rgb', hr)
+        _trace_mask('se.depth', hd)
+        pf, idx_f, pd, idx_d = Fn.stem_stage_fwd(y_rgb, y_depth, aff[0], aff[1], sr, sd)
+        ctx.set_materialize_grads(False)
+        ctx.save_for_backward(y_rgb, y_depth)
+        ctx.rts = (rt_rgb, rt_depth)
+        ctx.saved = (idx_f, idx_d, aff, st, (gr, hr, sr, flat(w1r), flat(w2r)),
+                     (gd, hd, sd, flat(w1d), flat(w2d)))
+        ctx.shapes = (w1r.shape, w2r.shape)
+        return pf, pd
+
+    @staticmethod
+    @once_differentiable
+    @_traced
+    def backward(ctx, g_f, g_d):
+        y_rgb, y_depth = ctx.saved_tensors
+        idx_f, idx_d, aff, st, se_r, se_d = ctx.saved
+        ctx.saved = None
+        rt_rgb, rt_depth = ctx.rts
+        n, c, h, w = y_rgb.shape
+        pooled = (n, (h + 1) // 2, (w + 1) // 2, c)
+
+        def grad(g):
+            if g is None:
+                return torch.zeros(pooled, device=y_rgb.device).permute(0, 3, 1, 2)
+            g = Fn.as_act(g, dense=True)
+            return g if g.dtype == torch.float32 else Fn.cast(g, torch.float32)
+        g_f, g_d = grad(g_f), grad(g_d)
+        sums, ds_r, ds_d = Fn.stem_stage_bwd_reduce(g_f, idx_f, g_d, idx_d, y_rgb, y_depth, aff[0],
+                                                    aff[1], st[0], st[1])
+        s1, s2 = ctx.shapes
+        se_grads, dgaps = [], []
+        for (gap, hid, s, w1, w2), ds in ((se_r, ds_r), (se_d, ds_d)):
+            dgap, dw1, db1, dw2, db2 = Fn.se_mlp_bwd(gap, w1, w2, hid, s, ds)
+            dgaps.append(dgap)
+            se_grads += [dw1.reshape(s1), db1, dw2.reshape(s2), db2]
+        tr, td = _bn_targets(rt_rgb.brt), _bn_targets(rt_depth.brt)
+        dgb = Fn.stem_stage_bwd_finalize(
+            sums, h * w, se_r[2], se_d[2], dgaps[0], dgaps[1],
+            (tr.get('dg_out'), tr.get('db_out')), (td.get('dg_out'), td.get('db_out')))
+        dy_rgb, dy_depth = Fn.stem_stage_bwd_apply(
+            g_f, idx_f, g_d, idx_d, y_rgb, y_depth, aff[0], aff[1], st[0], st[1],
+            rt_rgb.brt.bn.weight.detach(), rt_depth.brt.bn.weight.detach(), se_r[2], se_d[2],
+            dgaps[0], dgaps[1], dgb)
+        return (dy_rgb, None, dy_depth, None, None, None, dgb[0], dgb[1], dgb[2], dgb[3], *se_grads)
+
+
 class MaxPoolFunction(Function):
     @staticmethod
     def forward(ctx, x):
diff --git a/include/emsanet_hip.h b/include/emsanet_hip.h
--- a/include/emsanet_hip.h
+++ b/include/emsanet_hip.h
@@ -547,6 +547,45 @@
                        void* stream);
 int emsa_channel_mean_t(int32_t dtype, const void* x, float* gap, float* ws, int32_t n, int64_t
     hw, int32_t c, void* stream);
+int emsa_se_pair_mlp_fwd(const float* ws, const float* w1a, const float* b1a, const float* w2a,
+                         const float* b2a, const float* w1b, const float* b1b, const float* w2b,
+                         const float* b2b, float* gap, float* hid, float* s, int32_t n, int64_t hw,
+                         int32_t c, int32_t cr, void* stream);
+
+int emsa_stem_stage_squeeze(const float* y_rgb, const float* y_depth, const float* scale_rgb,
+                            const float* shift_rgb, const float* scale_depth,
+                            const float* shift_depth, float* ws, int32_t n, int64_t hw, int32_t c,
+                            void* stream);
+int emsa_stem_stage_fwd(const float* y_rgb, const float* y_depth, const float* scale_rgb,
+                        const float* shift_rgb, const float* scale_depth, const float* shift_depth,
+                        const float* s_rgb, const float* s_depth, float* pf, int8_t* idx_f,
+                        float* pd, int8_t* idx_d, int32_t n, int32_t h, int32_t w, int32_t c,
+                        void* stream);
+int emsa_stem_stage_bwd_splits(int32_t h, int32_t w);
+int emsa_stem_stage_bwd_reduce(const float* gf, const int8_t* idx_f, const float* gd,
+                               const int8_t* idx_d, const float* y_rgb, const float* y_depth,
+                               const float* scale_rgb, const float* shift_rgb,
+                               const float* scale_depth, const float* shift_depth,
+                               const float* mean_rgb, const float* invstd_rgb,
+                               const float* mean_depth, const float* invstd_depth, float* ws,
+                               double* sums, float* ds, int32_t n, int32_t h, int32_t w, int32_t c,
+                               void* stream);
+int emsa_stem_stage_bwd_finalize(const double* sums, const float* s_rgb, const float* s_depth,
+                                 const float* dgap_rgb, const float* dgap_depth, float* dgamma_rgb,
+                                 float* dbeta_rgb, float* dgamma_depth, float* dbeta_depth,
+                                 int32_t n, int64_t hw, int32_t c, void* stream);
+int emsa_stem_stage_bwd_apply(const float* gf, const int8_t* idx_f, const float* gd,
+                              const int8_t* idx_d, const float* y_rgb, const float* y_depth,
+                              const float* scale_rgb, const float* shift_rgb,
+                              const float* scale_depth, const float* shift_depth,
+                              const float* mean_rgb, const float* invstd_rgb,
+                              const float* mean_depth, const float* invstd_depth,
+                              const float* gamma_rgb, const float* gamma_depth, const float* s_rgb,
+                              const float* s_depth, const float* dgap_rgb, const float* dgap_depth,
+                              const float* dgamma_rgb, const float* dbeta_rgb,
+                              const float* dgamma_depth, const float* dbeta_depth, float* dy_rgb,
+                              float* dy_depth, int32_t n, int32_t h, int32_t w, int32_t c,
+                              void* stream);
 int emsa_se_scale_bwd_reduce_t(int32_t dtype, const void* dout, const void* x, float* ds, float*
     ws, int32_t n, int64_t hw, int32_t c, void* stream);
 int emsa_cast_channels(int32_t src_dtype, const void* x, int32_t ld_x, int32_t dst_dtype, void*
```

New measurement: 339.8 images/s, median of 6. 3.1% higher.
